# ZhangXiaze/DeepPointMap

Measured on AMD Instinct MI355X. Metric: LiDAR frames/s (encode+match+register), 65 536 pts/frame, higher is better.
Workload: dtype f32 (attention scores K Q^T and P V, Linear / Conv1d (+ LayerNorm) layers with K <= 2048 as exact three-way bf16 splits: 6 bf16 products per fp32 product, fp32 accumulate -- fp32 accuracy, bf16 matrix pipe; all else fp32); 1 GPU; synthetic 64x65536-pt scans per GPU: Encoder.forward + consecutive-frame registration_forward (256x256) + information matrix per frame; points_per_frame=65536, parallelism=frame-sharded x1, one RCCL gather of descriptors+edges per step, weights=procedural (deeppointmap_amd/weights.py), allocator_reserve_gib=16, geometry_waits_for_caller_stream=True

## Files before the change

### deeppointmap_amd/_lib.py

```python
from __future__ import annotations

import ctypes
import os

import torch
from ctypes import c_char_p, c_double, c_int, c_longlong, c_size_t, c_uint, c_void_p

_HERE = os.path.dirname(os.path.abspath(__file__))
LIB_PATH = os.environ.get("DPM_LIB") or os.path.join(_HERE, "libdpm_hip.so")
VERSION_EXPERIMENT = 0x40000000

P, I, D, LL = c_void_p, c_int, c_double, c_longlong

SIGNATURES = {
    "dpm_version": (I, []),
    "dpm_error_string": (c_char_p, [I]),
    "dpm_prepare_points": (I, [P, P, I, I, I, P, P, P]),
    "dpm_to_channel_first": (I, [P, I, I, I, P, P]),
    "dpm_to_channel_first_ld": (I, [P, I, I, I, P, I, P]),
    "dpm_emit_descriptors": (I, [P, P, P, I, I, I, D, P, P, P, P, P]),
    "dpm_nested_levels": (I, [P, P, I, I, I, P, P, P, P, P]),
    "dpm_gather_frames": (I, [P, LL, I, I, I, P, I, P, P]),
    "dpm_fps_workspace_bytes": (c_size_t, [I, I, I]),
    "dpm_fps": (I, [P, P, I, I, I, P, P, P, P, P]),
    "dpm_fps_ex": (I, [P, P, I, I, I, P, P, P, P, I, P]),
    "dpm_fps_start": (I, [P, P, P, I, I, I, P, P, P, P, P]),
    "dpm_knn_workspace_bytes": (c_size_t, [I, I]),
    "dpm_knn_hybrid": (I, [P, P, P, I, I, I, I, D, P, P, P]),
    "dpm_knn_hybrid_reuse": (I, [P, P, P, I, I, I, I, D, P, P, P, P, P]),
    "dpm_knn_build_grid": (I, [P, P, I, I, D, P, P]),
    "dpm_knn_hybrid_prebuilt": (I, [P, P, P, I, I, I, I, D, P, P, P]),
    "dpm_ball_query": (I, [P, P, P, I, I, I, I, D, P, P]),
    "dpm_voxel_sampler_bounds": (I, [P, P, I, I, I, D, D, P, P]),
    "dpm_voxel_sampler_workspace_bytes": (c_size_t, [I, I, LL]),
    "dpm_voxel_sampler_select": (I, [P, P, I, I, I, D, D, P, LL, I, P, I, P, P, P]),
    "dpm_posegraph_optimize": (I, [P, I, P, P, P, P, I, I, P, P, P]),
    "dpm_host_topk_replay": (I, [P, I, I, I, P]),
    "dpm_host_sort_replay": (I, [P, I, I, P]),
    "dpm_group_mlp_max": (I, [P, P, P, P, P, P, P, P, I, I, I, I, I, I, D, P, P]),
    "dpm_group_mlp_max_generic": (I, [P, P, P, P, P, P, P, P, I, I, I, I, I, I, D, P, P]),
    "dpm_group_mlp_max_from_xyz": (I, [P, P, P, P, P, P, P, P, P, I, I, I, I, I, I, D, P, P]),
    "dpm_group_gather_ln_max": (I, [P, P, P, P, P, I, P, P, I, I, I, I, I, D, P, P]),
    "dpm_group_gather_ln_max_folded": (I, [P, P, P, P, I, P, P, I, I, I, I, I, D, P, P]),
    "dpm_group_affine_ln_max": (I, [P, P, P, P, P, P, I, P, P, I, I, I, I, I, D, P, P]),
    "dpm_group_gather_ln_max_centred": (I, [P, P, P, P, I, P, P, I, I, I, I, I, D, P, P]),
    "dpm_group_affine_ln_max_centred": (I, [P, P, P, P, P, P, I, P, P, I, I, I, I, I, D, P, P]),
    "dpm_linear": (I, [P, I, P, I, P, P, I, P, I, I, I, I, I, P]),
    "dpm_linear_batched": (I, [P, I, LL, P, I, LL, P, P, I, LL, P, I, LL, I, I, I, I, I, P]),
    "dpm_split_bf16x3": (I, [P, LL, P, P]),
    "dpm_linear_bf16x3": (I, [P, I, P, I, LL, P, P, I, P, I, I, I, I, I, P]),
    "dpm_linear_bf16x3_rank3": (I, [P, I, P, I, LL, P, P, I, P, I, I, I, I, I, P, P, I, D, P]),
    "dpm_linear_layernorm_bf16x3": (I, [P, I, P, I, LL, P, P, P, P, P, P, I, I, I, I, I, P]),
    "dpm_pwconv_pair_bf16x3": (I, [P, I, P, LL, P, P, P, P, LL, P, P, P, P, P, I, I, I, P]),
    "dpm_decoder_tail_bf16x3": (I, [P, P, P, P, I, I, P, LL, P, P, P, P, LL, P, P, LL, P, P, P, P]),
    "dpm_layernorm": (I, [P, I, P, P, P, P, P, I, I, I, I, P]),
    "dpm_linear_layernorm": (I, [P, I, P, I, P, P, P, P, P, P, I, I, I, I, I, P]),
    "dpm_three_interp_cat": (I, [P, P, P, P, P, I, I, I, I, I, P, P]),
    "dpm_posemb": (I, [P, I, P, I, I, I, P, P]),
    "dpm_attention": (I, [P, I, LL, P, I, LL, P, I, LL, P, I, LL, I, I, I, I, I, P]),
    "dpm_attention_shifted": (I, [P, I, LL, P, I, LL, P, I, LL, P, I, LL, I, I, I, I, I, I, P]),
    "dpm_attention_masked": (I, [P, I, LL, P, I, LL, P, I, LL, P, I, LL, I, I, I, I, I, I, P, P]),
    "dpm_attention_indexed": (I, [P, I, LL, P, I, LL, P, I, LL, P, I, LL, I, I, I, I, I, I, P, P]),
    "dpm_attention_split_workspace_bytes": (c_size_t, [I, I, I, I, I]),
    "dpm_attention_planes_bytes": (c_size_t, [I, I, I]),
    "dpm_attention_planes": (I, [P, I, LL, P, P, I, LL, I, I, I, I, I, P, P]),
    "dpm_linear_bf16x3_kvplanes": (I, [P, I, P, I, LL, P, P, I, I, I, I, I, I, I, P, P]),
    "dpm_attention_split": (I, [P, I, LL, P, I, LL, P, I, LL, P, I, LL, I, I, I, I, I, I, I, P, P]),
    "dpm_l2_normalize": (I, [P, I, I, P, P]),
    "dpm_match_workspace_bytes": (c_size_t, [I, I, I, I]),
    "dpm_match_topk": (I, [P, P, I, I, I, I, D, I, P, P, P, P]),
    "dpm_pairing_workspace_bytes": (c_size_t, [I, I, I]),
    "dpm_dual_softmax_topk": (I, [P, I, I, I, D, I, P, P, P, P]),
    "dpm_gather_pairs": (I, [P, P, P, I, I, I, I, I, P, P, P, P]),
    "dpm_mean_rows": (I, [P, I, I, I, P, I, P]),
    "dpm_kabsch_workspace_bytes": (c_size_t, [I, I]),
    "dpm_corr_kabsch": (I, [P, P, I, LL, P, I, LL, P, P, P, I, I, D, I, D, P, P, P, I, P]),
    "dpm_preprocess_workspace_bytes": (c_size_t, [LL]),
    "dpm_preprocess_scan": (I, [P, I, I, D, D, D, D, LL, P, P, I, P, P, P]),
    "dpm_knn_self_workspace_bytes": (c_size_t, [I]),
    "dpm_knn_self": (I, [P, I, I, D, P, P, P, P, P]),
    "dpm_point_normals": (I, [P, I, D, P, P, P]),
    "dpm_lowpass_similarity": (I, [P, P, I, I, I, P, P]),
    "dpm_stat_filter": (I, [P, I, D, I, D, P, P, P, P, P, P]),
    "dpm_filter_dc_workspace_bytes": (c_size_t, [I, I]),
    "dpm_outlier_filter_dc": (I, [P, P, P, I, I, D, D, D, P, P, P, P, P]),
    "dpm_lowpass_filter_dc": (I, [P, P, P, I, D, I, D, I, D, D, P, P, P, P, P]),
    "dpm_augment_workspace_bytes": (c_size_t, [I, LL]),
    "dpm_ground_filter": (I, [P, P, P, I, I, I, D, D, I, P, P, P, P, P]),
    "dpm_voxel_select": (I, [P, P, P, I, D, I, LL, P, P, P, P, P]),
    "dpm_mask_select": (I, [P, P, P, I, I, D, D, P, D, P, I, P, P, P, P, P]),
    "dpm_points_affine": (I, [P, P, I, I, P, P, P]),
    "dpm_points_deskew": (I, [P, P, P, I, I, P, I, I, P, D, P]),
    "dpm_gather_points": (I, [P, P, P, I, P, I, I, P, P, P, P]),
    "dpm_pack_frames": (I, [P, P, P, I, I, P, P, P, P]),
    "dpm_ingest_frames": (I, [P, P, LL, I, I, I, P, P, P, P, P]),
    "dpm_map_tile": (I, [P, P, P, P, I, I, I, P, P]),
    "dpm_infomat_workspace_bytes": (c_size_t, [I, I, I]),
    "dpm_information_matrix": (I, [P, I, P, I, P, D, P, P, P]),
    "dpm_information_matrix_batched": (I, [P, I, P, P, I, P, I, D, P, I, P, P]),
    "dpm_infomat_build_grids": (I, [P, I, P, I, D, P, P]),
    "dpm_infomat_search_grids": (I, [P, I, P, P, I, P, I, D, P, I, P, P]),
    "dpm_icp_workspace_bytes": (c_size_t, [I, I]),
    "dpm_icp_refine_batched": (I, [P, I, I, P, P, P, P, I, P, I, P, P, I, D, D, P, P, P, P, P, P, P, P, P]),
    "dpm_voxel_map_workspace_bytes": (c_size_t, [LL]),
    "dpm_voxel_map_init": (I, [LL, P, P]),
    "dpm_voxel_map_bounds": (I, [P, P, P, I, LL, P, P]),
    "dpm_voxel_map_insert": (I, [P, P, P, I, LL, LL, LL, D, D, D, D, P, P]),
    "dpm_voxel_map_finish": (I, [LL, P, P]),
    "dpm_voxel_map_emit": (I, [P, LL, D, D, D, D, P, P, I, P]),
    "dpm_reg_loss_pairs": (I, [P, P, I, I, I, D, P, P, P, P, P]),
    "dpm_reg_loss_workspace_bytes": (c_size_t, [I, I, I, I]),
    "dpm_reg_loss_forward": (I, [P, P, P, P, P, P, P, P, I, I, I, I, D, D, I, P, P, P, P, P, P]),
    "dpm_reg_loss_backward": (I, [P, P, P, P, I, I, I, I, D, D, I, P, P, P, P, P, P]),
    "dpm_attention_train_workspace_bytes": (c_size_t, [I, I, I, I]),
    "dpm_attention_train_forward": (I, [P, I, LL, P, I, LL, P, I, LL, P, I, LL, P, I, I, I, I, I, P, P]),
    "dpm_attention_train_backward": (I, [P, I, LL, P, I, LL, P, I, LL, P, I, LL, P, P, I, LL, P, P, P, P, I, I, I, I, I, P, P]),
    "dpm_offset_pairs_count": (I, [P, P, P, P, I, I, I, D, P, P, P]),
    "dpm_offset_pairs_fill": (I, [P, P, P, P, I, I, I, D, P, P, P]),
    "dpm_offset_pairs_gather": (I, [P, I, P, I, I, LL, I, P, P]),
    "dpm_offset_pairs_segment_sum": (I, [P, I, P, P, LL, I, P, P]),
    "dpm_group_train_forward": (I, [P, P, P, P, P, I, P, P, I, I, I, I, I, D, P, P, P]),
    "dpm_group_train_workspace_bytes": (c_size_t, [I, I, I, I, I]),
    "dpm_group_train_backward": (I, [P, P, P, P, P, I, P, I, I, I, I, I, D, P, P, P, P, P, P, P, P]),
    "dpm_loop_pool_workspace_bytes": (c_size_t, [I, I, I]),
    "dpm_loop_pool_forward": (I, [P, I, P, P, I, I, I, P, P, P]),
    "dpm_loop_pool_backward": (I, [P, I, P, P, P, I, I, I, P, P, P, P]),
    "dpm_loop_bce_forward": (I, [P, P, I, P, P, P, P]),
    "dpm_dense_train_workspace_bytes": (c_size_t, [LL, I, I]),
    "dpm_dense_train_forward": (I, [P, I, P, I, P, P, P, P, P, LL, I, I, I, P, P, P, P]),
    "dpm_dense_train_backward_rows": (I, [P, P, P, P, P, LL, I, I, P, P, P, P, P, P]),
    "dpm_dense_train_backward_gemm": (I, [P, P, I, P, I, LL, I, I, P, P, P, P, P]),
    "dpm_map_poses": (I, [P, P, P, P, P, I, I, I, P, P, P]),
    "dpm_map_assemble_fwd": (I, [P, P, P, P, P, I, I, I, I, I, D, P, P, P, P, P, P, P]),
    "dpm_map_assemble_bwd": (I, [P, P, I, I, I, I, I, P, P]),
    "dpm_optim_chunk": (I, []),
    "dpm_optim_step": (I, [I, P, P, I, D, D, D, D, D, D, D, D, I, I, P]),
    "dpm_flat_pack": (I, [P, P, I, P, LL, P]),
    "dpm_flat_unpack": (I, [P, P, I, P, LL, P]),
    "dpm_optim_step_synced": (I, [I, P, P, I, D, D, D, D, D, D, D, D, I, I, P, I, LL, D, P]),
    "dpm_lidar_cull": (I, [P, P, I, P, P, I, D, I, P, P, P, P]),
    "dpm_lidar_cast": (I, [P, P, P, I, I, P, I, I, D, D, P, P, P, P]),
    "dpm_lidar_cull_sweep": (I, [P, P, I, P, P, P, I, I, D, I, P, P, P, P, P]),
    "dpm_lidar_cast_sweep": (I, [P, P, P, I, I, P, I, I, P, I, D, D, P, P, P, P]),
    "dpm_lidar_emit": (I, [P, P, P, P, I, I, P, P, D, P, P, I, P, P, P, P, P, P]),
    "dpm_scene_distance": (I, [P, I, P, I, D, I, D, D, D, P, P, P]),
    "dpm_cloud_nn_workspace_bytes": (c_size_t, [I, I]),
    "dpm_cloud_nn": (I, [P, I, P, I, D, D, D, D, P, P, P, P]),
    "dpm_distance_stats_workspace_bytes": (c_size_t, [I, I, I]),
    "dpm_distance_stats": (I, [P, I, P, P, I, I, P, I, D, P, P, P]),
    "dpm_local_map_bytes": (c_size_t, [I, I]),
    "dpm_local_map_init": (I, [P, I, I, P]),
    "dpm_local_map_insert": (I, [P, I, I, I, D, P, P, P, P, I, P, c_uint, D, D, P]),
    "dpm_local_map_prune": (I, [P, I, I, I, D, P, P, D, P]),
    "dpm_local_map_insert_frames": (I, [P, I, I, I, D, P, P, P, I, I, P, P, P, I, P, D, D, D, P]),
    "dpm_local_map_register": (I, [P, I, I, I, D, P, P, P, I, P, P, P, I, D, D, D, P, P, P, P, P, P, P, P, P, P]),
    "dpm_local_map_export": (I, [P, I, I, I, P, P, P, P, P, I, P]),
    "dpm_local_map_planes": (I, [P, I, I, I, D, P, D, P, P, P]),
    "dpm_local_map_register_planes": (I, [P, I, I, I, D, P, P, P, I, D, P, P, I, P, P, P, I, D, D, D, P, P, P, P, P, P, P, P, P,
                                          P]),
    "dpm_tsdf_bytes": (c_size_t, [I]),
    "dpm_tsdf_init": (I, [P, I, P]),
    "dpm_tsdf_integrate": (I, [P, I, D, P, P, P, I, P, D, D, D, D, P]),
    "dpm_tsdf_integrate_frames": (I, [P, I, D, P, P, P, I, I, P, P, I, D, D, D, D, P]),
    "dpm_tsdf_integrate_planes": (I, [P, I, D, P, P, P, P, I, P, D, D, D, D, D, P]),
    "dpm_tsdf_integrate_planes_frames": (I, [P, I, D, P, P, P, P, I, I, P, P, I, D, D, D, D, D, P]),
    "dpm_tsdf_carve": (I, [P, I, D, P, P, P, I, P, D, D, D, D, I, D, P]),
    "dpm_tsdf_carve_frames": (I, [P, I, D, P, P, P, I, I, P, P, I, D, D, D, D, I, D, P]),
    "dpm_tsdf_export": (I, [P, I, P, P, P, P, I, P]),
    "dpm_tsdf_surface": (I, [P, I, D, I, P, P, P, P, P, I, P]),
    "dpm_tsdf_mesh": (I, [P, I, D, I, P, P, P, P, I, P]),
    "dpm_tsdf_sample": (I, [P, I, D, P, P, P, I, P, I, P, P, P, P]),
    "dpm_tsdf_register_scratch_bytes": (c_size_t, [I]),
    "dpm_tsdf_register": (I, [P, I, D, P, D, I, D, P, P, I, P, P, P, I, D, D, D, P, P, P, P, P, P, P, P, P]),
    "dpm_tsdf_blocks_bytes": (c_size_t, [I]),
    "dpm_tsdf_blocks": (I, [P, I, I, P, I, P]),
    "dpm_tsdf_raycast": (I, [P, I, D, P, P, I, P, I, P, I, D, D, D, I, P, P, P, P]),
    "dpm_scan_context_build": (I, [P, P, I, I, I, D, D, D, P, P, P, P, P, P]),
    "dpm_scan_context_build_batched": (I, [P, P, I, I, I, I, D, D, D, P, P, P, P, P, P]),
    "dpm_scan_context_search_workspace_bytes": (c_size_t, [I, I, I]),
    "dpm_scan_context_search": (I, [P, P, I, P, P, I, P, I, I, I, P, P, P, P, P]),
}


class DpmError(RuntimeError):
    pass


_lib = None


def load() -> ctypes.CDLL:
    global _lib
    if _lib is None:
        if not os.path.exists(LIB_PATH):
            raise DpmError(
                f"{LIB_PATH} not found: the HIP extension is not built. "
                "Run `python deeppointmap_amd/csrc/build.py` (there is no CPU fallback)."
            )
        lib = ctypes.CDLL(LIB_PATH)
        for name, (res, args) in SIGNATURES.items():
            fn = getattr(lib, name)
            fn.restype, fn.argtypes = res, args
        if lib.dpm_version() & VERSION_EXPERIMENT:
            import sys
            print(f"deeppointmap_amd: {LIB_PATH} is an EXPERIMENTAL build (-DDPM_EXPERIMENT): its kernels read DPM_* "
                  "measurement switches from the environment, some of which skip work -- not for results", file=sys.stderr)
        _lib = lib
# ... 15 lines not shown
```

### deeppointmap_amd/csrc/build.py

```python
#!/usr/bin/env python3
import os
import subprocess
import sys
from concurrent.futures import ThreadPoolExecutor

HERE = os.path.dirname(os.path.abspath(__file__))
OUT = os.path.join(os.path.dirname(HERE), "libdpm_hip.so")
ARCH = "gfx950"
COMMON = ["--offload-arch=" + ARCH, "-O3", "-std=c++17", "-fPIC", "-Wall", "-Wno-unused-function",
          "-ffp-contract=off", "-Xclang", "-target-feature", "-Xclang", "-packed-fp32-ops"]
SOURCES = {
    "fps.hip": [],
    "fps_tree.hip": [],
    "knn.hip": [],
    "encoder_ops.hip": [],
    "gemm.hip": [],
    "gemm_b3.hip": [],
    "group_mlp.hip": [],
    "decoder_ops.hip": [],
    "match.hip": [],
    "infomat.hip": [],
    "icp.hip": [],
    "preprocess.hip": [],
    "voxel_sample.hip": [],
    "posegraph.hip": [],
    "voxel_map.hip": [],
    "reg_loss.hip": [],
    "attention_train.hip": [],
    "offset_pairs.hip": [],
    "group_train.hip": [],
    "loop_head_train.hip": [],
    "dense_train.hip": [],
    "augment.hip": [],
    "map_assemble.hip": [],
    "optim.hip": [],
    "ingest.hip": [],
    "lidar_sim.hip": [],
    "map_eval.hip": [],
    "deskew.hip": [],
    "gn_one.hip": [],
    "local_map.hip": [],
    "scan_context.hip": [],
    "tsdf_map.hip": [],
}


def _stale(target, deps):
    if not os.path.exists(target):
        return True
    t = os.path.getmtime(target)
    return any(os.path.getmtime(d) > t for d in deps)


def build(force=False, verbose=False, flags=(), out=None, only=None):
    hipcc = os.environ.get("HIPCC", "/opt/rocm/bin/hipcc")
    objdir = os.path.join(HERE, "build") if out is None else os.path.join(HERE, "build", os.path.basename(out) + ".d")
    OUT = globals()["OUT"] if out is None else out
    os.makedirs(objdir, exist_ok=True)
    headers = [os.path.join(HERE, h) for h in os.listdir(HERE) if h.endswith(".h")]
    headers.append(os.path.join(os.path.dirname(os.path.dirname(HERE)), "include", "dpm_hip.h"))
    jobs = []
    for src, extra in SOURCES.items():
        s = os.path.join(HERE, src)
        o = os.path.join(objdir, src.replace(".hip", ".o"))
        if force or _stale(o, [s] + headers):
            jobs.append([hipcc, *COMMON, *extra, *(flags if only is None or src in only else ()), "-c", s, "-o", o])

    def run(cmd):
        if verbose:
            print(" ".join(cmd), flush=True)
        subprocess.check_call(cmd)

    with ThreadPoolExecutor(max_workers=4) as ex:
        list(ex.map(run, jobs))
    objs = [os.path.join(objdir, s.replace(".hip", ".o")) for s in SOURCES]
    if force or jobs or _stale(OUT, objs):
        staged = OUT + ".unlinted"
        run([hipcc, "--offload-arch=" + ARCH, "-shared", "-fPIC", "-o", staged, *objs])
        sys.path.insert(0, HERE)
        import isa_lint
        try:
            if out is None:
                isa_lint.check(staged)
            elif verbose:
                print("packed fp32 instructions:", isa_lint.packed_fp32(staged))
        except BaseException:
            os.remove(staged)
            raise
        os.replace(staged, OUT)
    return OUT


def build_abi_smoke(verbose=False):
    hipcc = os.environ.get("HIPCC", "/opt/rocm/bin/hipcc")
    root = os.path.dirname(os.path.dirname(HERE))
    src = os.path.join(root, "tests", "c", "abi_gpu_smoke.cpp")
    exe = os.path.join(HERE, "build", "abi_gpu_smoke")
    if not os.path.exists(src):
        return None
    if _stale(exe, [src, OUT, os.path.join(root, "include", "dpm_hip.h")]):
        cmd = [hipcc, "--offload-arch=" + ARCH, "-O2", "-ffp-contract=off", "-I" + os.path.join(root, "include"), src, "-o", exe,
               "-L" + os.path.dirname(OUT), "-ldpm_hip", "-Wl,-rpath,$ORIGIN/../.."]
        if verbose:
            print(" ".join(cmd), flush=True)
        subprocess.check_call(cmd)
    return exe


if __name__ == "__main__":
    if "--out" in sys.argv:
        i = sys.argv.index("--out")
        rest, only = sys.argv[i + 2:], None
        if rest[:1] == ["--only"]:
            only, rest = set(rest[1].split(",")), rest[2:]
            assert only <= set(SOURCES), only
        print(build(verbose=True, flags=tuple(rest), out=os.path.abspath(sys.argv[i + 1]), only=only))
        sys.exit(0)
    print(build(force="--force" in sys.argv, verbose=True))
    print(build_abi_smoke(verbose=True))
```

### deeppointmap_amd/csrc/gemm_b3.hip

```cpp
#include "dpm_common.h"
#include <type_traits>

namespace {

using bf16x8 = __attribute__((ext_vector_type(8))) __bf16;
using f32x4 = __attribute__((ext_vector_type(4))) float;
using u32x4 = __attribute__((ext_vector_type(4))) unsigned;
using u32x2 = __attribute__((ext_vector_type(2))) unsigned;

__device__ __forceinline__ float b3_act(float v, int act) {
    if (act == DPM_ACT_RELU) return fmaxf(v, 0.f);
    if (act == DPM_ACT_SIGMOID) return 1.f / (1.f + __expf(-v));
    return v;
}

__global__ __launch_bounds__(256) void split_bf16x3_kernel(const float *__restrict__ W, long long n, uint16_t *__restrict__ planes) {
    const long long i = (long long)blockIdx.x * 256 + threadIdx.x;
    if (i >= n) return;
    unsigned h, m, l;
    split3(W[i], h, m, l);
    planes[i] = (uint16_t)(h >> 16), planes[n + i] = (uint16_t)(m >> 16), planes[2 * n + i] = (uint16_t)(l >> 16);
}

#ifndef DPM_B3_WIDE
#define DPM_B3_WIDE 1024
#endif
#ifndef DPM_B3_DEEP
#define DPM_B3_DEEP 256
#endif
constexpr int B3_KT = 32, B3_LD = B3_KT;

struct KvPlanes {
    uint16_t *p;
    int col0, tokens, heads;
};

template <int BM, int BN, bool XVEC, int PF, bool KVP>
__device__ __forceinline__ void gemm_b3_body(const float *__restrict__ X, int ldx, const uint16_t *__restrict__ Wp, int ldw,
                                             long long plane, const float *__restrict__ bias,
                                             const float *__restrict__ res, int ldr, float *__restrict__ out, int ldo,
                                             int R, int Cin, int Cout, int act, const float *__restrict__ r3x,
                                             const float *__restrict__ r3w, int ldr3, float r3s, KvPlanes kv) {
    constexpr int LDC = BN + 4, MB = BM / 32, NB = BN / 32, PX = BM / 32, WT = BN * 4, PW = (WT + 255) / 256;
    constexpr int SM0 = 3 * (BM + BN) * B3_LD, SM1 = 2 * BM * LDC, SM = SM0 > SM1 ? SM0 : SM1;
    __shared__ __attribute__((aligned(16))) uint16_t smem[SM];
    uint16_t (*Xs)[BM][B3_LD] = reinterpret_cast<uint16_t (*)[BM][B3_LD]>(smem);
    uint16_t (*Ws)[BN][B3_LD] = reinterpret_cast<uint16_t (*)[BN][B3_LD]>(smem + 3 * BM * B3_LD);
    const int t = threadIdx.x, lane = t & 63, w = t >> 6, wm = w >> 1, wn = w & 1;
    int by = blockIdx.y, bx = blockIdx.x;
    if ((gridDim.y & 7) == 0 && gridDim.y >= 64) {
        const unsigned L = blockIdx.y * gridDim.x + blockIdx.x, xcd = L & 7, slot = L >> 3;
        by = (int)((slot / gridDim.x) * 8 + xcd), bx = (int)(slot % gridDim.x);
    }
    const int row0 = by * BM, col0 = bx * BN;
    const int xr_ = t >> 3, xk = (t & 7) * 4, wr_ = min(t >> 2, BN - 1), wk = (t & 3) * 8;
    const float *xp[PX];
#pragma unroll
    for (int p = 0; p < PX; ++p) xp[p] = X + (size_t)min(row0 + p * 32 + xr_, R - 1) * ldx + xk;
    const uint16_t *wp[PW];
#pragma unroll
    for (int p = 0; p < PW; ++p) wp[p] = Wp + (size_t)min(col0 + p * 64 + wr_, Cout - 1) * ldw + wk;
    auto load_x = [&](const float *p) {
        if (XVEC) return *reinterpret_cast<const f32x4 *>(p);
        return f32x4{p[0], p[1], p[2], p[3]};
    };
    f32x4 xv[PF][PX];
    u32x4 wv[PF][PW][3];
#pragma unroll
    for (int d = 0; d < PF; ++d) {
        const int kd = min(d * B3_KT, Cin - B3_KT);
#pragma unroll
        for (int p = 0; p < PX; ++p) xv[d][p] = load_x(xp[p] + kd);
#pragma unroll
        for (int p = 0; p < PW; ++p)
#pragma unroll
            for (int pl = 0; pl < 3; ++pl) wv[d][p][pl] = *reinterpret_cast<const u32x4 *>(wp[p] + pl * plane + kd);
    }
    f32x4 acc[MB][NB];
#pragma unroll
    for (int i = 0; i < MB; ++i)
#pragma unroll
        for (int j = 0; j < NB; ++j) acc[i][j] = f32x4{0.f, 0.f, 0.f, 0.f};
    const int fr = lane & 15, fk = (lane >> 4) * 8;
    auto stage_x = [&](const f32x4 &v, int r) {
        unsigned h0, m0, l0, h1, m1, l1, h2, m2, l2, h3, m3, l3;
        split3(v[0], h0, m0, l0), split3(v[1], h1, m1, l1), split3(v[2], h2, m2, l2), split3(v[3], h3, m3, l3);
        *reinterpret_cast<u32x2 *>(&Xs[0][r][b3_col(r, xk)]) = u32x2{pack2(h0, h1), pack2(h2, h3)};
        *reinterpret_cast<u32x2 *>(&Xs[1][r][b3_col(r, xk)]) = u32x2{pack2(m0, m1), pack2(m2, m3)};
        *reinterpret_cast<u32x2 *>(&Xs[2][r][b3_col(r, xk)]) = u32x2{pack2(l0, l1), pack2(l2, l3)};
    };
    for (int kb = 0; kb < Cin; kb += B3_KT * PF)
#pragma unroll
    for (int d = 0; d < PF; ++d) {
        const int k0 = kb + d * B3_KT;
        if (PF > 1 && k0 >= Cin) break;
#pragma unroll
        for (int p = 0; p < PX; ++p) stage_x(xv[d][p], p * 32 + xr_);
        if (WT >= 256 || t < WT) {
#pragma unroll
            for (int p = 0; p < PW; ++p)
#pragma unroll
                for (int pl = 0; pl < 3; ++pl) *reinterpret_cast<u32x4 *>(&Ws[pl][p * 64 + wr_][b3_col(wr_, wk)]) = wv[d][p][pl];
        }
        __syncthreads();
        {
            const int kn = min(k0 + PF * B3_KT, Cin - B3_KT);
#pragma unroll
            for (int p = 0; p < PX; ++p) xv[d][p] = load_x(xp[p] + kn);
#pragma unroll
            for (int p = 0; p < PW; ++p)
#pragma unroll
                for (int pl = 0; pl < 3; ++pl) wv[d][p][pl] = *reinterpret_cast<const u32x4 *>(wp[p] + pl * plane + kn);
        }
        bf16x8 a[3][NB], b[3][MB];
#pragma unroll
        for (int pl = 0; pl < 3; ++pl) {
#pragma unroll
            for (int j = 0; j < NB; ++j) a[pl][j] = *reinterpret_cast<const bf16x8 *>(&Ws[pl][wn * (BN / 2) + j * 16 + fr][b3_col(fr, fk)]);
#pragma unroll
            for (int i = 0; i < MB; ++i) b[pl][i] = *reinterpret_cast<const bf16x8 *>(&Xs[pl][wm * (BM / 2) + i * 16 + fr][b3_col(fr, fk)]);
        }
#define DPM_B3(PWQ, PXQ)                                                                                   \
    _Pragma("unroll") for (int i = 0; i < MB; ++i) _Pragma("unroll") for (int j = 0; j < NB; ++j)        \
        acc[i][j] = __builtin_amdgcn_mfma_f32_16x16x32_bf16(a[PWQ][j], b[PXQ][i], acc[i][j], 0, 0, 0)
        DPM_B3(1, 1);
        DPM_B3(2, 0);
        DPM_B3(0, 2);
        DPM_B3(1, 0);
        DPM_B3(0, 1);
        DPM_B3(0, 0);
#undef DPM_B3
        __syncthreads();
    }
    float *ct = reinterpret_cast<float *>(smem);
#pragma unroll
    for (int i = 0; i < MB; ++i)
#pragma unroll
        for (int j = 0; j < NB; ++j)
            *reinterpret_cast<float4 *>(&ct[(wm * (BM / 2) + i * 16 + (lane & 15)) * LDC + wn * (BN / 2) + j * 16 + (lane >> 4) * 4]) =
                make_float4(acc[i][j][0], acc[i][j][1], acc[i][j][2], acc[i][j][3]);
    __syncthreads();
    if (KVP && BM == 64 && BN % 32 == 0 && col0 >= kv.col0) {
        const int E = kv.heads * 32, colk = col0 - kv.col0, isV = colk >= E ? 1 : 0, head0 = (colk - isV * E) >> 5;
        const int sq_ = row0 / kv.tokens, kt = (row0 - sq_ * kv.tokens) >> 6, ntile = kv.tokens >> 6;
#pragma unroll 1
        for (int hh = 0; hh < BN / 32; ++hh) {
            uint16_t *img = kv.p + ((((size_t)sq_ * kv.heads + head0 + hh) * ntile + kt) * 2 + isV) * 6144;
            const float *bh = bias ? bias + col0 + hh * 32 : nullptr;
#pragma unroll
            for (int p = 0; p < 2; ++p) {
                const int e = t + p * 256;
                if (!isV) {
                    const int kr = e >> 3, c4 = (e & 7) * 4;
                    float4 v = *reinterpret_cast<const float4 *>(&ct[kr * LDC + hh * 32 + c4]);
                    if (bh) {
                        const float4 bv = *reinterpret_cast<const float4 *>(bh + c4);
                        v.x += bv.x, v.y += bv.y, v.z += bv.z, v.w += bv.w;
                    }
                    unsigned h0, m0, l0, h1, m1, l1, h2, m2, l2, h3, m3, l3;
                    split3(v.x, h0, m0, l0), split3(v.y, h1, m1, l1), split3(v.z, h2, m2, l2), split3(v.w, h3, m3, l3);
                    uint16_t *o = img + kr * 32 + b3_col(kr, c4);
                    *reinterpret_cast<u32x2 *>(o) = u32x2{pack2(h0, h1), pack2(h2, h3)};
                    *reinterpret_cast<u32x2 *>(o + 2048) = u32x2{pack2(m0, m1), pack2(m2, m3)};
                    *reinterpret_cast<u32x2 *>(o + 4096) = u32x2{pack2(l0, l1), pack2(l2, l3)};
                } else {
                    const int d = e & 31, slot0 = (e >> 5) * 4;
                    const int key0 = 32 * (slot0 >> 5) + 16 * ((slot0 & 7) >> 2) + 4 * ((slot0 >> 3) & 3);
                    const float b = bh ? bh[d] : 0.f;
                    unsigned hq[4], mq[4], lq[4];
#pragma unroll
                    for (int q = 0; q < 4; ++q) split3(ct[(key0 + q) * LDC + hh * 32 + d] + b, hq[q], mq[q], lq[q]);
                    uint16_t *o = img + d * 64 + (((((slot0 >> 3) ^ (d >> 1)) & 7) << 3) | (slot0 & 7));
                    *reinterpret_cast<u32x2 *>(o) = u32x2{pack2(hq[0], hq[1]), pack2(hq[2], hq[3])};
                    *reinterpret_cast<u32x2 *>(o + 2048) = u32x2{pack2(mq[0], mq[1]), pack2(mq[2], mq[3])};
                    *reinterpret_cast<u32x2 *>(o + 4096) = u32x2{pack2(lq[0], lq[1]), pack2(lq[2], lq[3])};
                }
            }
        }
        return;
    }
    constexpr int TPR = BN / 4, RPS = 256 / TPR;
    const int cr = t / TPR, cc = (t % TPR) * 4, c = col0 + cc;
    if (c < Cout) {
// ... 50 lines not shown
template <int BM, int BN, int WGM, int WGN>
__global__ __launch_bounds__(64 * WGM * WGN) void gemm_ln_b3_kernel(const float *__restrict__ X, int ldx, const uint16_t *__restrict__ Wp,
                                                                   int ldw, long long plane, const float *__restrict__ bias,
                                                                   const float *__restrict__ pre, const float *__restrict__ gamma,
                                                                   const float *__restrict__ beta, const float *__restrict__ post,
                                                                   float *__restrict__ out, int ldo, int R, int Cin, int act) {
    constexpr int NP = 1;
    constexpr int BNP = BN / NP;
    constexpr int T = 64 * WGM * WGN, WM = BM / WGM, WN = BNP / WGN, MB = WM / 16, NB = WN / 16, LDC = BN + 4;
    constexpr int XF = BM * 8, PX = (XF + T - 1) / T;
    constexpr int WF = BNP * 4, PW = (WF + T - 1) / T;
    constexpr int SM0 = 3 * (BM + BNP) * B3_LD, SM1 = 2 * BM * LDC, SM = SM0 > SM1 ? SM0 : SM1;
    static_assert(MB >= 1 && NB >= 1 && BN % NP == 0 && WM % 16 == 0 && WN % 16 == 0, "tile shape");
    __shared__ __attribute__((aligned(16))) uint16_t smem[SM];
    uint16_t (*Xs)[BM][B3_LD] = reinterpret_cast<uint16_t (*)[BM][B3_LD]>(smem);
    uint16_t (*Ws)[BNP][B3_LD] = reinterpret_cast<uint16_t (*)[BNP][B3_LD]>(smem + 3 * BM * B3_LD);
    const int t = threadIdx.x, lane = t & 63, w = t >> 6, wm = w / WGN, wn = w % WGN;
    const int row0 = blockIdx.x * BM;
    const float *xp[PX];
    int xrow[PX], xk[PX];
#pragma unroll
    for (int p = 0; p < PX; ++p) {
        const int g = min(p * T + t, XF - 1);
        xrow[p] = g >> 3, xk[p] = (g & 7) * 4;
        xp[p] = X + (size_t)min(row0 + xrow[p], R - 1) * ldx + xk[p];
    }
    const uint16_t *wp[PW];
    int wrow[PW], wk[PW];
#pragma unroll
    for (int p = 0; p < PW; ++p) {
        const int g = min(p * T + t, WF - 1);
        wrow[p] = g >> 2, wk[p] = (g & 3) * 8;
        wp[p] = Wp + (size_t)wrow[p] * ldw + wk[p];
    }
    f32x4 xv[PX];
    u32x4 wv[PW][3];
#pragma unroll
    for (int p = 0; p < PX; ++p) xv[p] = *reinterpret_cast<const f32x4 *>(xp[p]);
#pragma unroll
    for (int p = 0; p < PW; ++p)
#pragma unroll
        for (int pl = 0; pl < 3; ++pl) wv[p][pl] = *reinterpret_cast<const u32x4 *>(wp[p] + pl * plane);
    f32x4 acc[NP][MB][NB];
#pragma unroll
    for (int ps = 0; ps < NP; ++ps)
#pragma unroll
        for (int i = 0; i < MB; ++i)
#pragma unroll
            for (int j = 0; j < NB; ++j) acc[ps][i][j] = f32x4{0.f, 0.f, 0.f, 0.f};
    const int fr = lane & 15, fk = (lane >> 4) * 8;
#pragma unroll
    for (int ps = 0; ps < NP; ++ps)
    for (int k0 = 0; k0 < Cin; k0 += B3_KT) {
#pragma unroll
        for (int p = 0; p < PX; ++p) {
            if (XF % T == 0 || p * T + t < XF) {
                unsigned h0, m0, l0, h1, m1, l1, h2, m2, l2, h3, m3, l3;
                split3(xv[p][0], h0, m0, l0), split3(xv[p][1], h1, m1, l1), split3(xv[p][2], h2, m2, l2), split3(xv[p][3], h3, m3, l3);
                *reinterpret_cast<u32x2 *>(&Xs[0][xrow[p]][b3_col(xrow[p], xk[p])]) = u32x2{pack2(h0, h1), pack2(h2, h3)};
                *reinterpret_cast<u32x2 *>(&Xs[1][xrow[p]][b3_col(xrow[p], xk[p])]) = u32x2{pack2(m0, m1), pack2(m2, m3)};
                *reinterpret_cast<u32x2 *>(&Xs[2][xrow[p]][b3_col(xrow[p], xk[p])]) = u32x2{pack2(l0, l1), pack2(l2, l3)};
            }
        }
#pragma unroll
        for (int p = 0; p < PW; ++p) {
            if (WF % T == 0 || p * T + t < WF) {
#pragma unroll
                for (int pl = 0; pl < 3; ++pl) *reinterpret_cast<u32x4 *>(&Ws[pl][wrow[p]][b3_col(wrow[p], wk[p])]) = wv[p][pl];
            }
        }
        __syncthreads();
        {
            const bool wrap = k0 + B3_KT >= Cin && ps + 1 < NP;
            const int kn = wrap ? 0 : min(k0 + B3_KT, Cin - B3_KT);
            const size_t wo = (size_t)(wrap ? ps + 1 : ps) * BNP * ldw + kn;
#pragma unroll
            for (int p = 0; p < PX; ++p) xv[p] = *reinterpret_cast<const f32x4 *>(xp[p] + kn);
#pragma unroll
            for (int p = 0; p < PW; ++p)
#pragma unroll
                for (int pl = 0; pl < 3; ++pl) wv[p][pl] = *reinterpret_cast<const u32x4 *>(wp[p] + pl * plane + wo);
        }
        bf16x8 a[3][NB], b[3][MB];
#pragma unroll
        for (int pl = 0; pl < 3; ++pl) {
#pragma unroll
            for (int j = 0; j < NB; ++j) a[pl][j] = *reinterpret_cast<const bf16x8 *>(&Ws[pl][wn * WN + j * 16 + fr][b3_col(fr, fk)]);
#pragma unroll
            for (int i = 0; i < MB; ++i) b[pl][i] = *reinterpret_cast<const bf16x8 *>(&Xs[pl][wm * WM + i * 16 + fr][b3_col(fr, fk)]);
        }
#define DPM_B3(PWQ, PXQ)                                                                                   \
    _Pragma("unroll") for (int i = 0; i < MB; ++i) _Pragma("unroll") for (int j = 0; j < NB; ++j)        \
        acc[ps][i][j] = __builtin_amdgcn_mfma_f32_16x16x32_bf16(a[PWQ][j], b[PXQ][i], acc[ps][i][j], 0, 0, 0)
        DPM_B3(1, 1);
        DPM_B3(2, 0);
        DPM_B3(0, 2);
        DPM_B3(1, 0);
        DPM_B3(0, 1);
        DPM_B3(0, 0);
#undef DPM_B3
        __syncthreads();
    }
    float *ct = reinterpret_cast<float *>(smem);
#pragma unroll
    for (int ps = 0; ps < NP; ++ps)
#pragma unroll
        for (int i = 0; i < MB; ++i)
#pragma unroll
            for (int j = 0; j < NB; ++j)
                *reinterpret_cast<float4 *>(&ct[(wm * WM + i * 16 + (lane & 15)) * LDC + ps * BNP + wn * WN + j * 16 + (lane >> 4) * 4]) =
                    make_float4(acc[ps][i][j][0], acc[ps][i][j][1], acc[ps][i][j][2], acc[ps][i][j][3]);
    __syncthreads();
    constexpr int G = BN / 4, RPS = T / G;
    const int cr = t / G, cc = (t % G) * 4;
    const float4 bv = bias ? *reinterpret_cast<const float4 *>(bias + cc) : make_float4(0.f, 0.f, 0.f, 0.f);
    const float4 g4 = *reinterpret_cast<const float4 *>(gamma + cc), b4 = *reinterpret_cast<const float4 *>(beta + cc);
    auto gsum = [](float v) {
#pragma unroll
        for (int off = 1; off < G; off <<= 1) v += __shfl_xor(v, off, 64);
        return v;
    };
#pragma unroll 4
    for (int p = 0; p < BM / RPS; ++p) {
        const int r = row0 + p * RPS + cr, rr = min(r, R - 1);
        float4 v = *reinterpret_cast<const float4 *>(&ct[(p * RPS + cr) * LDC + cc]);
        v.x += bv.x, v.y += bv.y, v.z += bv.z, v.w += bv.w;
        if (pre) {
            const float4 pv = *reinterpret_cast<const float4 *>(pre + (size_t)rr * BN + cc);
            v.x += pv.x, v.y += pv.y, v.z += pv.z, v.w += pv.w;
        }
        const float mu = gsum((v.x + v.y) + (v.z + v.w)) / (float)BN;
        v.x -= mu, v.y -= mu, v.z -= mu, v.w -= mu;
        const float rs = rsqrtf(gsum(fmaf(v.x, v.x, fmaf(v.y, v.y, fmaf(v.z, v.z, v.w * v.w)))) / (float)BN + 1e-5f);
        float4 o = make_float4(fmaf(v.x * rs, g4.x, b4.x), fmaf(v.y * rs, g4.y, b4.y), fmaf(v.z * rs, g4.z, b4.z),
                               fmaf(v.w * rs, g4.w, b4.w));
        if (post) {
            const float4 pv = *reinterpret_cast<const float4 *>(post + (size_t)rr * BN + cc);
            o.x += pv.x, o.y += pv.y, o.z += pv.z, o.w += pv.w;
        }
        o.x = b3_act(o.x, act), o.y = b3_act(o.y, act), o.z = b3_act(o.z, act), o.w = b3_act(o.w, act);
        if (r < R) *reinterpret_cast<float4 *>(out + (size_t)r * ldo + cc) = o;
    }
}

struct TailArgs {
    const float *a, *pre, *post;
    float *out;
    const uint16_t *w[3];
    long long plane[3];
    const float *bias[3];
    const float *g2, *be2, *g3, *be3;
    int R;
};
constexpr int DT_BM = 64, DT_C = 256, DT_T = 512, DT_NK = DT_C / B3_KT, DT_LDC = DT_C + 4;
#ifndef DPM_TAIL_STASH
#define DPM_TAIL_STASH 2
#endif
constexpr int DT_NS = DPM_TAIL_STASH, DT_OPER = 3 * (DT_BM + DT_C) * B3_LD;
__device__ __forceinline__ f32x4 *dt_stash(uint16_t *smem, int kt) {
    return reinterpret_cast<f32x4 *>(smem + DT_OPER) + (kt - (DT_NK - DT_NS)) * DT_T + threadIdx.x;
}
__device__ __forceinline__ void dt_stash_put(uint16_t *smem, const f32x4 (&v)[DT_NK]) {
#pragma unroll
    for (int kt = DT_NK - DT_NS; kt < DT_NK; ++kt) *dt_stash(smem, kt) = v[kt];
}

template <typename V, typename P>
__device__ __forceinline__ V *dt_at(P *uniform, unsigned bytes) {
    using B = std::conditional_t<std::is_const<P>::value, const char, char>;
    return reinterpret_cast<V *>(reinterpret_cast<B *>(uniform) + bytes);
}
__device__ __forceinline__ long long dt_uniform(long long o) {
    const unsigned lo = __builtin_amdgcn_readfirstlane((unsigned)o), hi = __builtin_amdgcn_readfirstlane((unsigned)((unsigned long long)o >> 32));
    return (long long)(((unsigned long long)hi << 32) | lo);
}
template <int CTRL>
__device__ __forceinline__ float dt_dpp(float v) {
    return __int_as_float(__builtin_amdgcn_update_dpp(__float_as_int(v), __float_as_int(v), CTRL, 0xF, 0xF, false));
}
__device__ __forceinline__ float dt_row_sum(float (&s)[DT_NK]) {
#pragma unroll
    for (int kt = 0; kt < DT_NK; ++kt) {
        s[kt] += dt_dpp<0xB1>(s[kt]);
        s[kt] += dt_dpp<0x4E>(s[kt]);
        s[kt] += dt_dpp<0x141>(s[kt]);
    }
    return ((s[0] + s[1]) + (s[2] + s[3])) + ((s[4] + s[5]) + (s[6] + s[7]));
}
__device__ __forceinline__ void dt_layernorm(f32x4 (&v)[DT_NK], const float *__restrict__ gamma, const float *__restrict__ beta, int sk) {
    float s[DT_NK];
#pragma unroll
    for (int kt = 0; kt < DT_NK; ++kt) s[kt] = (v[kt][0] + v[kt][1]) + (v[kt][2] + v[kt][3]);
    const float mu = dt_row_sum(s) / (float)DT_C;
#pragma unroll
    for (int kt = 0; kt < DT_NK; ++kt) {
        v[kt][0] -= mu, v[kt][1] -= mu, v[kt][2] -= mu, v[kt][3] -= mu;
        s[kt] = fmaf(v[kt][0], v[kt][0], fmaf(v[kt][1], v[kt][1], fmaf(v[kt][2], v[kt][2], v[kt][3] * v[kt][3])));
    }
    const float rs = rsqrtf(dt_row_sum(s) / (float)DT_C + 1e-5f);
#pragma unroll
    for (int kt = 0; kt < DT_NK; ++kt) {
        const f32x4 g4 = *reinterpret_cast<const f32x4 *>(gamma + kt * B3_KT + sk), b4 = *reinterpret_cast<const f32x4 *>(beta + kt * B3_KT + sk);
#pragma unroll
        for (int q = 0; q < 4; ++q) v[kt][q] = fmaf(v[kt][q] * rs, g4[q], b4[q]);
    }
}

__device__ __forceinline__ const u32x4 *dt_wsrc(const uint16_t *__restrict__ Wp, long long plane, int p, int pl, int k0, unsigned wo) {
    return dt_at<const u32x4>(Wp + dt_uniform(pl * plane + p * (DT_T / 4) * DT_C) + k0, wo);
}
__device__ __forceinline__ unsigned dt_woff() { return (unsigned)((threadIdx.x >> 2) * DT_C + (threadIdx.x & 3) * 8) * 2u; }
__device__ __forceinline__ void dt_wtile0(const uint16_t *__restrict__ Wp, long long plane, u32x4 (&wv)[2][3]) {
    const unsigned wo = dt_woff();
#pragma unroll
    for (int p = 0; p < 2; ++p)
#pragma unroll
        for (int pl = 0; pl < 3; ++pl) wv[p][pl] = *dt_wsrc(Wp, plane, p, pl, 0, wo);
}

template <bool XREG, typename Mid>
__device__ __forceinline__ void dt_product(uint16_t *smem, const float *xg, unsigned xo, const f32x4 (&xr)[DT_NK], const uint16_t *__restrict__ Wp,
                                           long long plane, u32x4 (&wv)[2][3], f32x4 (&acc)[2][4], Mid mid) {
    constexpr int WM = 32, WN = 64, MB = 2, NB = 4, PW = 2;
    uint16_t (*Xs)[DT_BM][B3_LD] = reinterpret_cast<uint16_t (*)[DT_BM][B3_LD]>(smem);
    uint16_t (*Ws)[DT_C][B3_LD] = reinterpret_cast<uint16_t (*)[DT_C][B3_LD]>(smem + 3 * DT_BM * B3_LD);
    const int t = threadIdx.x, lane = t & 63, w = t >> 6, wm = w >> 2, wn = w & 3;
    const int sr = t >> 3, sk = (t & 7) * 4, wk = (t & 3) * 8, fr = lane & 15, fk = (lane >> 4) * 8;
    const int wrow = t >> 2;
    const unsigned wo = dt_woff();
    f32x4 xv = f32x4{0.f, 0.f, 0.f, 0.f};
    if (!XREG) xv = *dt_at<const f32x4>(xg, xo);
#pragma unroll
    for (int i = 0; i < MB; ++i)
#pragma unroll
        for (int j = 0; j < NB; ++j) acc[i][j] = f32x4{0.f, 0.f, 0.f, 0.f};
#pragma unroll
    for (int kt = 0; kt < DT_NK; ++kt) {
        {
            const f32x4 x = !XREG ? xv : kt >= DT_NK - DT_NS ? *dt_stash(smem, kt) : xr[kt];
            unsigned h0, m0, l0, h1, m1, l1, h2, m2, l2, h3, m3, l3;
            split3(x[0], h0, m0, l0), split3(x[1], h1, m1, l1), split3(x[2], h2, m2, l2), split3(x[3], h3, m3, l3);
            *reinterpret_cast<u32x2 *>(&Xs[0][sr][b3_col(sr, sk)]) = u32x2{pack2(h0, h1), pack2(h2, h3)};
            *reinterpret_cast<u32x2 *>(&Xs[1][sr][b3_col(sr, sk)]) = u32x2{pack2(m0, m1), pack2(m2, m3)};
            *reinterpret_cast<u32x2 *>(&Xs[2][sr][b3_col(sr, sk)]) = u32x2{pack2(l0, l1), pack2(l2, l3)};
        }
#pragma unroll
        for (int p = 0; p < PW; ++p)
#pragma unroll
            for (int pl = 0; pl < 3; ++pl) *reinterpret_cast<u32x4 *>(&Ws[pl][p * (DT_T / 4) + wrow][b3_col(wrow, wk)]) = wv[p][pl];
        __syncthreads();
        if (kt + 1 < DT_NK) {
            const int kn = (kt + 1) * B3_KT;
            unsigned wok = wo;
            asm volatile("" : "+v"(wok));
            if (!XREG) xv = *dt_at<const f32x4>(xg + kn, xo);
#pragma unroll
            for (int p = 0; p < PW; ++p)
#pragma unroll
                for (int pl = 0; pl < 3; ++pl) wv[p][pl] = *dt_wsrc(Wp, plane, p, pl, kn, wok);
        }
        mid(kt);
        bf16x8 b[3][MB];
#pragma unroll
        for (int pl = 0; pl < 3; ++pl)
#pragma unroll
            for (int i = 0; i < MB; ++i) b[pl][i] = *reinterpret_cast<const bf16x8 *>(&Xs[pl][wm * WM + i * 16 + fr][b3_col(fr, fk)]);
#pragma unroll
        for (int j = 0; j < NB; ++j) {
            bf16x8 a[3];
#pragma unroll
            for (int pl = 0; pl < 3; ++pl) a[pl] = *reinterpret_cast<const bf16x8 *>(&Ws[pl][wn * WN + j * 16 + fr][b3_col(fr, fk)]);
#define DPM_B3(PWQ, PXQ) \
    _Pragma("unroll") for (int i = 0; i < MB; ++i) acc[i][j] = __builtin_amdgcn_mfma_f32_16x16x32_bf16(a[PWQ], b[PXQ][i], acc[i][j], 0, 0, 0)
            DPM_B3(1, 1);
            DPM_B3(2, 0);
            DPM_B3(0, 2);
            DPM_B3(1, 0);
            DPM_B3(0, 1);
            DPM_B3(0, 0);
#undef DPM_B3
        }
        __syncthreads();
    }
}

template <typename Mid>
__device__ __forceinline__ void dt_restage(uint16_t *smem, const f32x4 (&acc)[2][4], f32x4 (&v)[DT_NK], Mid mid) {
    float *ct = reinterpret_cast<float *>(smem);
    int t = threadIdx.x;
    asm volatile("" : "+v"(t));
    const int lane = t & 63, w = t >> 6, wm = w >> 2, wn = w & 3, sr = t >> 3, sk = (t & 7) * 4;
#pragma unroll
    for (int i = 0; i < 2; ++i)
#pragma unroll
        for (int j = 0; j < 4; ++j)
            *reinterpret_cast<f32x4 *>(&ct[(wm * 32 + i * 16 + (lane & 15)) * DT_LDC + wn * 64 + j * 16 + (lane >> 4) * 4]) = acc[i][j];
    mid();
    __syncthreads();
#pragma unroll
    for (int kt = 0; kt < DT_NK; ++kt) v[kt] = *reinterpret_cast<const f32x4 *>(&ct[sr * DT_LDC + kt * B3_KT + sk]);
    __syncthreads();
}

__device__ __forceinline__ void dt_add_bias(f32x4 (&v)[DT_NK], const float *__restrict__ bias, int sk) {
#pragma unroll
    for (int kt = 0; kt < DT_NK; ++kt) {
        const f32x4 bv = bias ? *reinterpret_cast<const f32x4 *>(bias + kt * B3_KT + sk) : f32x4{0.f, 0.f, 0.f, 0.f};
        v[kt] += bv;
    }
}

template <bool ZREG>
__global__ __launch_bounds__(DT_T) __attribute__((amdgpu_waves_per_eu(4, 4))) void decoder_tail_b3_kernel(TailArgs A) {
    constexpr int SM0 = DT_OPER + DT_NS * DT_T * 8, SM1 = 2 * DT_BM * DT_LDC, SM = SM0 > SM1 ? SM0 : SM1;
    __shared__ __attribute__((aligned(16))) uint16_t smem[SM];
    const int t = threadIdx.x, sr = t >> 3, sk = (t & 7) * 4;
    const int row0 = blockIdx.x * DT_BM, r = row0 + sr;
    const long long base = dt_uniform((long long)row0 * DT_C);
    const unsigned ro = (unsigned)(min(sr, A.R - 1 - row0) * DT_C + sk) * 4u;
    const float *ga = A.a + base, *gpre = A.pre + base, *gpost = (A.post ? A.post : A.pre) + base;
    float *gout = A.out + base;
    f32x4 acc[2][4], v[DT_NK], z[DT_NK];
    u32x4 wv[2][3];
    dt_wtile0(A.w[0], A.plane[0], wv);
    dt_product<false>(smem, ga, ro, v, A.w[0], A.plane[0], wv, acc, [&](int kt) {
        if (kt == DT_NK - 1) {
#pragma unroll
            for (int k2 = 0; k2 < DT_NK; ++k2) z[k2] = *dt_at<const f32x4>(gpre + k2 * B3_KT, ro);
        }
    });
    dt_restage(smem, acc, v, [&] { dt_wtile0(A.w[1], A.plane[1], wv); });
    dt_add_bias(v, A.bias[0], sk);
#pragma unroll
    for (int kt = 0; kt < DT_NK; ++kt) v[kt] += z[kt];
    dt_layernorm(v, A.g2, A.be2, sk);
    if (ZREG) {
#pragma unroll
        for (int kt = 0; kt < DT_NK; ++kt) z[kt] = v[kt];
    } else if (r < A.R) {
#pragma unroll
        for (int kt = 0; kt < DT_NK; ++kt) *dt_at<f32x4>(gout + kt * B3_KT, ro) = v[kt];
    }
    dt_stash_put(smem, v);
    dt_product<true>(smem, nullptr, 0u, v, A.w[1], A.plane[1], wv, acc, [](int) {});
    dt_restage(smem, acc, v, [&] { dt_wtile0(A.w[2], A.plane[2], wv); });
    dt_add_bias(v, A.bias[1], sk);
#pragma unroll
    for (int kt = 0; kt < DT_NK; ++kt)
#pragma unroll
        for (int q = 0; q < 4; ++q) v[kt][q] = fmaxf(v[kt][q], 0.f);
    dt_stash_put(smem, v);
    dt_product<true>(smem, nullptr, 0u, v, A.w[2], A.plane[2], wv, acc, [&](int kt) {
        if (!ZREG && kt == DT_NK - 1) {
#pragma unroll
            for (int k2 = 0; k2 < DT_NK; ++k2) z[k2] = *dt_at<const f32x4>(gout + k2 * B3_KT, ro);
        }
    });
    f32x4 pv[DT_NK];
    dt_restage(smem, acc, v, [&] {
        if (A.post) {
#pragma unroll
            for (int kt = 0; kt < DT_NK; ++kt) pv[kt] = *dt_at<const f32x4>(gpost + kt * B3_KT, ro);
        }
    });
    dt_add_bias(v, A.bias[2], sk);
#pragma unroll
    for (int kt = 0; kt < DT_NK; ++kt) v[kt] += z[kt];
    dt_layernorm(v, A.g3, A.be3, sk);
    if (A.post) {
#pragma unroll
        for (int kt = 0; kt < DT_NK; ++kt) v[kt] += pv[kt];
    }
    if (r < A.R) {
#pragma unroll
        for (int kt = 0; kt < DT_NK; ++kt) *dt_at<f32x4>(gout + kt * B3_KT, ro) = v[kt];
    }
}


#ifndef DPM_PW_GRID
#define DPM_PW_GRID 768
#endif
constexpr int PW_C = 32, PW_H = 128;
__device__ __forceinline__ float pw_rows4_sum(float v) {
    auto a = __builtin_amdgcn_permlane32_swap(__float_as_uint(v), __float_as_uint(v), false, false);
    v = __uint_as_float(a[0]) + __uint_as_float(a[1]);
    auto b = __builtin_amdgcn_permlane16_swap(__float_as_uint(v), __float_as_uint(v), false, false);
    return __uint_as_float(b[0]) + __uint_as_float(b[1]);
}
__global__ __launch_bounds__(256) void pwconv_pair_b3_kernel(const float *__restrict__ X, int ldx, const uint16_t *__restrict__ W1p,
                                                            long long plane1, const float *__restrict__ b1,
                                                            const float *__restrict__ g1, const float *__restrict__ be1,
                                                            const uint16_t *__restrict__ W2p, long long plane2,
                                                            const float *__restrict__ b2, const float *__restrict__ g2,
                                                            const float *__restrict__ be2, const float *__restrict__ post,
                                                            float *__restrict__ out, int R, int tiles_per_wave) {
    __shared__ __attribute__((aligned(16))) uint16_t W1s[3][PW_H][PW_C];
    __shared__ __attribute__((aligned(16))) uint16_t W2s[3][PW_H / 32][PW_C][32];
    __shared__ __attribute__((aligned(16))) float vec1[3][PW_H];
    __shared__ __attribute__((aligned(16))) float vec2[3][PW_C];
    const int t = threadIdx.x, lane = t & 63, w = t >> 6, g = lane >> 4, fr = lane & 15;
    for (int e = t; e < 3 * PW_H * 4; e += 256) {
        const int pl = e / (PW_H * 4), r = (e / 4) % PW_H, c = (e & 3) * 8;
        *reinterpret_cast<u32x4 *>(&W1s[pl][r][b3_col(r, c)]) = *reinterpret_cast<const u32x4 *>(W1p + pl * plane1 + r * PW_C + c);
    }
    for (int e = t; e < 3 * PW_C * 16; e += 256) {
        const int pl = e / (PW_C * 16), r = (e / 16) % PW_C, c = (e & 15) * 8;
        *reinterpret_cast<u32x4 *>(&W2s[pl][c >> 5][r][b3_col(r, c & 31)]) =
            *reinterpret_cast<const u32x4 *>(W2p + pl * plane2 + r * PW_H + c);
    }
    if (t < PW_H) vec1[0][t] = b1 ? b1[t] : 0.f, vec1[1][t] = g1[t], vec1[2][t] = be1[t];
    if (t < PW_C) vec2[0][t] = b2 ? b2[t] : 0.f, vec2[1][t] = g2[t], vec2[2][t] = be2[t];
    __syncthreads();
    const long long tile0 = ((long long)blockIdx.x * 4 + w) * tiles_per_wave;
    f32x4 nx0, nx1, np0, np1;
    auto request = [&](long long r0) {
        const int r = (int)min(r0 + fr, (long long)R - 1);
        const float *xp = X + (size_t)r * ldx + 8 * g;
        nx0 = *reinterpret_cast<const f32x4 *>(xp), nx1 = *reinterpret_cast<const f32x4 *>(xp + 4);
        np0 = post ? *reinterpret_cast<const f32x4 *>(post + (size_t)r * PW_C + 4 * g) : f32x4{0.f, 0.f, 0.f, 0.f};
        np1 = post ? *reinterpret_cast<const f32x4 *>(post + (size_t)r * PW_C + 16 + 4 * g) : f32x4{0.f, 0.f, 0.f, 0.f};
    };
    request(min(tile0 * 16, (long long)R - 1));
    for (int it = 0; it < tiles_per_wave; ++it) {
        const long long row0 = (tile0 + it) * 16;
        if (row0 >= R) break;
        const int row = (int)min(row0 + fr, (long long)R - 1);
        const f32x4 x0 = nx0, x1 = nx1, p0 = np0, p1 = np1;
        request(min(row0 + 16, (long long)R - 1));
        bf16x8 xb[3];
        {
            unsigned hh[8], mm[8], ll[8];
#pragma unroll
            for (int e = 0; e < 4; ++e) split3(x0[e], hh[e], mm[e], ll[e]), split3(x1[e], hh[4 + e], mm[4 + e], ll[4 + e]);
            xb[0] = __builtin_bit_cast(bf16x8, u32x4{pack2(hh[0], hh[1]), pack2(hh[2], hh[3]), pack2(hh[4], hh[5]), pack2(hh[6], hh[7])});
            xb[1] = __builtin_bit_cast(bf16x8, u32x4{pack2(mm[0], mm[1]), pack2(mm[2], mm[3]), pack2(mm[4], mm[5]), pack2(mm[6], mm[7])});
            xb[2] = __builtin_bit_cast(bf16x8, u32x4{pack2(ll[0], ll[1]), pack2(ll[2], ll[3]), pack2(ll[4], ll[5]), pack2(ll[6], ll[7])});
        }
        f32x4 h[PW_H / 16];
#pragma unroll
        for (int j = 0; j < PW_H / 16; j += 2) {
            bf16x8 a[2][3];
#pragma unroll
            for (int jj = 0; jj < 2; ++jj)
#pragma unroll
                for (int pl = 0; pl < 3; ++pl)
                    a[jj][pl] = *reinterpret_cast<const bf16x8 *>(&W1s[pl][(j + jj) * 16 + fr][b3_col(fr, 8 * g)]);
            h[j] = h[j + 1] = f32x4{0.f, 0.f, 0.f, 0.f};
#define DPM_PW1(PWQ, PXQ)                                                                             \
    _Pragma("unroll") for (int jj = 0; jj < 2; ++jj)                                                  \
        h[j + jj] = __builtin_amdgcn_mfma_f32_16x16x32_bf16(a[jj][PWQ], xb[PXQ], h[j + jj], 0, 0, 0)
            DPM_PW1(1, 1);
            DPM_PW1(2, 0);
            DPM_PW1(0, 2);
            DPM_PW1(1, 0);
            DPM_PW1(0, 1);
            DPM_PW1(0, 0);
#undef DPM_PW1
        }
        float sum = 0.f;
#pragma unroll
        for (int j = 0; j < PW_H / 16; ++j) {
            const f32x4 bv = *reinterpret_cast<const f32x4 *>(&vec1[0][16 * j + 4 * g]);
// ... 210 lines not shown
```

### deeppointmap_amd/decoder.py

```python
from __future__ import annotations

import copy
import threading
from typing import Dict, Tuple, Union

import torch
import torch.nn.functional as F
from torch.utils.checkpoint import checkpoint

from . import knobs, ops
from .params import ParamTree, decoder_shapes

HEADS = 8


class Decoder(ParamTree):
    def __init__(self, args):
        super().__init__(decoder_shapes(args))
        self.args = args
        self.decoder_cfg = args.decoder
        self.in_channel = self.decoder_cfg.in_channel
        self.model_channel = self.decoder_cfg.model_channel
        self.attention_layers = self.decoder_cfg.attention_layers
        self.tau = args.loss.tau
        self._dim_t: Dict[str, torch.Tensor] = {}
        self.fused_match = knobs.FUSED_MATCH
        self.stack_sides = True
        self.dedup_frames = knobs.DEDUP_FRAMES
        self.graph_min_hits = 2
        self.graph_max = 6
        self._graphs: Dict[tuple, dict] = {}
        self._graph_lock = threading.Lock()
        self._stamp_params = None
        self.train_checkpoint_rows = 8192
        self.eval()

    def __deepcopy__(self, memo):
        new = self.__class__.__new__(self.__class__)
        memo[id(self)] = new
        for k, v in self.__dict__.items():
            if k == "_graphs":
                new.__dict__[k] = {}
            elif k == "_stamp_params":
                new.__dict__[k] = None
            elif k == "_graph_lock":
                new.__dict__[k] = threading.Lock()
            else:
                new.__dict__[k] = copy.deepcopy(v, memo)
        return new

    @property
    def device(self) -> torch.device:
        return self.p("projection.weight").device

    def _dimt(self, dev: torch.device) -> torch.Tensor:
        key = str(dev)
        if key not in self._dim_t:
            F = self.model_channel // 3 // 2 * 2
            i = torch.arange(F, dtype=torch.float32)
            self._dim_t[key] = (10000 ** (2 * torch.div(i, 2, rounding_mode="trunc") / F)).to(dev)
        return self._dim_t[key]

    def _lin(self, key: str, x, act=ops.ACT_NONE, residual=None):
        return ops.linear(x, self.p(key + ".weight"), self.p(key + ".bias"), act=act, residual=residual)

    def _ln(self, key: str, x, post=None):
        return ops.layernorm(x, self.p(key + ".weight"), self.p(key + ".bias"), post=post)

    def _lin_ln(self, lin: str, ln: str, x, residual, post=None):
        return ops.linear_layernorm(x, self.p(lin + ".weight"), self.p(lin + ".bias"), self.p(ln + ".weight"),
                                    self.p(ln + ".bias"), pre=residual, post=post)

    def _block_tail(self, pre: str, a, z1, post=None):
        ca, n2, m0, m2, n3 = pre + ".cross_attn.out_proj", pre + ".norm2", pre + ".mlp.0", pre + ".mlp.2", pre + ".norm3"
        out = ops.decoder_tail(a, z1, self.p(ca + ".weight"), self.p(ca + ".bias"), self.p(n2 + ".weight"), self.p(n2 + ".bias"),
                               self.p(m0 + ".weight"), self.p(m0 + ".bias"), self.p(m2 + ".weight"), self.p(m2 + ".bias"),
                               self.p(n3 + ".weight"), self.p(n3 + ".bias"), post)
        if out is not None:
            return out
        z2 = self._lin_ln(ca, n2, a, z1)
        return self._lin_ln(m2, n3, self._lin(m0, z2, ops.ACT_RELU), z2, post)

    def _stage(self, desc: torch.Tensor, dev) -> Tuple[torch.Tensor, torch.Tensor, int, int]:
        d = desc.to(device=dev, dtype=torch.float32).contiguous()
        B, C, M = d.shape
        if C != self.in_channel + 3:
            raise ValueError(f"descriptor must have {self.in_channel + 3} rows, got {C}")
        t = ops.to_channel_first(d, row_multiple=4)
        return t.as_strided((B * M, C), (t.stride(1), 1), t.storage_offset()), B, M

    def _self_attn(self, pre: str, xp, B, M, norm: str = None, post=None, mask=None):
        E = self.model_channel
        a = ops.qkv_attention(xp, self.p(pre + ".in_proj_weight"), self.p(pre + ".in_proj_bias"), B, M, HEADS) if mask is None else None
        if a is None:
            qkv = ops.linear(xp, self.p(pre + ".in_proj_weight"), self.p(pre + ".in_proj_bias"))
            a = ops.attention(qkv[:, :E], qkv[:, E:2 * E], qkv[:, 2 * E:], B, M, M, HEADS, key_mask=mask)
        if norm is not None:
            return self._lin_ln(pre + ".out_proj", norm, a, xp, post)
        return ops.linear(a, self.p(pre + ".out_proj.weight"), self.p(pre + ".out_proj.bias"), residual=xp)

    def _cross_attn(self, pre: str, xq, xkv, B, M, N, norm: str = None, mask=None, tail=None):
        E = self.model_channel
        w, b = self.p(pre + ".in_proj_weight"), self.p(pre + ".in_proj_bias")
        q = ops.linear(xq, w[:E], b[:E])
        kv = ops.linear(xkv, w[E:], b[E:])
        a = ops.attention(q, kv[:, :E], kv[:, E:], B, M, N, HEADS, key_mask=mask)
        if tail is not None:
            return self._block_tail(tail[0], a, xq, tail[1])
        if norm is not None:
            return self._lin_ln(pre + ".out_proj", norm, a, xq)
        return ops.linear(a, self.p(pre + ".out_proj.weight"), self.p(pre + ".out_proj.bias"), residual=xq)

    def _descriptor_attention_forward(self, src_descriptor, dst_descriptor, src_padding_mask=None,
                                      dst_padding_mask=None):
        dev = self.device
        ts, B, M = self._stage(src_descriptor, dev)
        td, B2, N = self._stage(dst_descriptor, dev)
        if B != B2:
            raise ValueError("src and dst batch sizes differ")
        ms = md = None
        if src_padding_mask is not None or dst_padding_mask is not None:
            def as_mask(m, L):
                if m is None:
                    return torch.zeros(B, L, dtype=torch.uint8, device=dev)
                m = m.to(dev)
                if tuple(m.shape) != (B, L) or m.dtype != torch.bool:
                    raise ValueError(f"padding mask must be a bool tensor of shape ({B}, {L})")
                return m.contiguous().view(torch.uint8)
            ms, md = as_mask(src_padding_mask, M), as_mask(dst_padding_mask, N)
        C, E = self.in_channel, self.model_channel
        xyz_s, xyz_d = ts[:, C:C + 3], td[:, C:C + 3]
        if M == N:
            x, y = self._attention_layers_joint(ts, td, B, M, mask=None if ms is None else torch.cat([ms, md]))
            return x, xyz_s, y, xyz_d, B, M, N
        if self.stack_sides:
            x, y = self._attention_layers_stacked(ts, td, B, M, N, ms, md)
            return x, xyz_s, y, xyz_d, B, M, N
        ps, pd = ops.posemb(xyz_s, self._dimt(dev), E), ops.posemb(xyz_d, self._dimt(dev), E)
        xp = ops.linear(ts[:, :C], self.p("projection.weight"), self.p("projection.bias"), residual=ps)
        yp = ops.linear(td[:, :C], self.p("projection.weight"), self.p("projection.bias"), residual=pd)
        for l in range(self.attention_layers):
            pre = f"descriptor_attention.{l}"
            last = l == self.attention_layers - 1
            x1 = self._self_attn(pre + ".self_attn", xp, B, M, norm=pre + ".norm1", post=ps, mask=ms)
            y1 = self._self_attn(pre + ".self_attn", yp, B, N, norm=pre + ".norm1", post=pd, mask=md)
            xp = self._cross_attn(pre + ".cross_attn", x1, y1, B, M, N, mask=md, tail=(pre, None if last else ps))
            yp = self._cross_attn(pre + ".cross_attn", y1, x1, B, N, M, mask=ms, tail=(pre, None if last else pd))
        return xp, xyz_s, yp, xyz_d, B, M, N

    def _attention_layers_stacked(self, ts, td, B, M, N, ms=None, md=None):
        C, E, dev = self.in_channel, self.model_channel, self.device
        R1 = B * M
        z_in = torch.cat([ts, td], dim=0)
        pos = ops.posemb(z_in[:, C:C + 3], self._dimt(dev), E)
        zp = ops.linear(z_in[:, :C], self.p("projection.weight"), self.p("projection.bias"), residual=pos)
        for l in range(self.attention_layers):
            pre = f"descriptor_attention.{l}"
            last = l == self.attention_layers - 1
            sa, ca = pre + ".self_attn", pre + ".cross_attn"
            qkv = ops.linear(zp, self.p(sa + ".in_proj_weight"), self.p(sa + ".in_proj_bias"))
            a = torch.empty(zp.shape[0], E, device=dev, dtype=torch.float32)
            ops.attention(qkv[:R1, :E], qkv[:R1, E:2 * E], qkv[:R1, 2 * E:], B, M, M, HEADS, out=a[:R1], key_mask=ms)
            ops.attention(qkv[R1:, :E], qkv[R1:, E:2 * E], qkv[R1:, 2 * E:], B, N, N, HEADS, out=a[R1:], key_mask=md)
            z1 = self._lin_ln(sa + ".out_proj", pre + ".norm1", a, zp, pos)
            qkv = ops.linear(z1, self.p(ca + ".in_proj_weight"), self.p(ca + ".in_proj_bias"))
            a = torch.empty(zp.shape[0], E, device=dev, dtype=torch.float32)
            ops.attention(qkv[:R1, :E], qkv[R1:, E:2 * E], qkv[R1:, 2 * E:], B, M, N, HEADS, out=a[:R1], key_mask=md)
            ops.attention(qkv[R1:, :E], qkv[:R1, E:2 * E], qkv[:R1, 2 * E:], B, N, M, HEADS, out=a[R1:], key_mask=ms)
            zp = self._block_tail(pre, a, z1, None if last else pos)
        return zp[:R1], zp[R1:]

    def _attention_layers_joint(self, ts, td, B, M, frames=None, mask=None):
        C, E, R = self.in_channel, self.model_channel, B * M
        dev = self.device
        if frames is not None:
            tu, sidx, didx = frames
            U = tu.shape[0] // M
            pos_u = ops.posemb(tu[:, C:C + 3], self._dimt(dev), E)
            zu = ops.linear(tu[:, :C], self.p("projection.weight"), self.p("projection.bias"), residual=pos_u)
            pre = "descriptor_attention.0"
            z1u = self._self_attn(pre + ".self_attn", zu, U, M, norm=pre + ".norm1", post=pos_u)
            order = sidx if didx is None else torch.cat([sidx, didx])
            pos = ops.gather_frames(pos_u, order, M, E).view(2 * R, E)
            z1_first = ops.gather_frames(z1u, order, M, E).view(2 * R, E)
            ca0 = pre + ".cross_attn"
            a_first = qkv_u = None
            if self.dedup_frames and E // HEADS == 32 and mask is None:
                a_first = ops.qkv_attention(z1u, self.p(ca0 + ".in_proj_weight"), self.p(ca0 + ".in_proj_bias"), 2 * B, M, HEADS,
                                            kv_shift=B, seq_index=order)
                if a_first is None:
                    qkv_u = ops.linear(z1u, self.p(ca0 + ".in_proj_weight"), self.p(ca0 + ".in_proj_bias"))
            zp = None
        else:
            z_in = torch.cat([ts, td], dim=0)
            pos = ops.posemb(z_in[:, C:C + 3], self._dimt(dev), E)
            zp = ops.linear(z_in[:, :C], self.p("projection.weight"), self.p("projection.bias"), residual=pos)
            z1_first = qkv_u = a_first = None
        for l in range(self.attention_layers):
            pre = f"descriptor_attention.{l}"
            last = l == self.attention_layers - 1
            if l == 0 and z1_first is not None:
                z1 = z1_first
            else:
                z1 = self._self_attn(pre + ".self_attn", zp, 2 * B, M, norm=pre + ".norm1", post=pos, mask=mask)
            ca = pre + ".cross_attn"
            if l == 0 and z1_first is not None and a_first is not None:
                a = a_first
            elif l == 0 and z1_first is not None and qkv_u is not None:
                a = ops.attention(qkv_u[:, :E], qkv_u[:, E:2 * E], qkv_u[:, 2 * E:], 2 * B, M, M, HEADS, kv_shift=B,
                                  seq_index=order)
            else:
                a = ops.qkv_attention(z1, self.p(ca + ".in_proj_weight"), self.p(ca + ".in_proj_bias"), 2 * B, M, HEADS,
                                      kv_shift=B) if mask is None else None
                if a is None:
                    qkv = ops.linear(z1, self.p(ca + ".in_proj_weight"), self.p(ca + ".in_proj_bias"))
                    a = ops.attention(qkv[:, :E], qkv[:, E:2 * E], qkv[:, 2 * E:], 2 * B, M, M, HEADS, kv_shift=B, key_mask=mask)
            zp = self._block_tail(pre, a, z1, None if last else pos)
        return zp[:R], zp[R:]

    def train(self, mode: bool = True):
        was = self.training
        super().train(mode)
        loop = self.train_stage == "loop_detection"
        for name, p in self._flat.items():
            p.requires_grad_(bool(mode) and (("loop" in name) == loop))
        if was and not mode:
            self.invalidate_caches()
        return self

    def _train_layer(self, l: int, z, pos, B: int, M: int, N: int, ms, md):
        E, R1 = self.model_channel, B * M
        pre = f"descriptor_attention.{l}"
        nrm = lambda n: (self.p(f"{pre}.{n}.weight"), self.p(f"{pre}.{n}.bias"))
        zp = z + pos
        qkv = self._dense(zp, self.p(pre + ".self_attn.in_proj_weight"), self.p(pre + ".self_attn.in_proj_bias"))
        a = torch.cat([ops.attention_train(qkv[:R1, :E], qkv[:R1, E:2 * E], qkv[:R1, 2 * E:], B, M, M, HEADS, ms),
                       ops.attention_train(qkv[R1:, :E], qkv[R1:, E:2 * E], qkv[R1:, 2 * E:], B, N, N, HEADS, md)])
        z1 = self._dense_ln(a, *self._w(pre + ".self_attn.out_proj"), *nrm("norm1"), residual=zp, post=pos)
        qkv = self._dense(z1, self.p(pre + ".cross_attn.in_proj_weight"), self.p(pre + ".cross_attn.in_proj_bias"))
        a = torch.cat([ops.attention_train(qkv[:R1, :E], qkv[R1:, E:2 * E], qkv[R1:, 2 * E:], B, M, N, HEADS, md),
                       ops.attention_train(qkv[R1:, :E], qkv[:R1, E:2 * E], qkv[:R1, 2 * E:], B, N, M, HEADS, ms)])
        z2 = self._dense_ln(a, *self._w(pre + ".cross_attn.out_proj"), *nrm("norm2"), residual=z1)
        u = self._dense(z2, *self._w(pre + ".mlp.0"), act=ops.ACT_RELU)
        return self._dense_ln(u, *self._w(pre + ".mlp.2"), *nrm("norm3"), residual=z2)

    def _dense2(self, x, first: str, second: str):
        return self._dense(self._dense(x, *self._w(first), act=ops.ACT_RELU), *self._w(second))

    def forward(self, src_descriptor: torch.Tensor, dst_descriptor: torch.Tensor, src_padding_mask: torch.Tensor = None,
                dst_padding_mask: torch.Tensor = None, gt_Rt: Tuple[torch.Tensor, torch.Tensor] = None):
        assert self.training, "forward is not available during inference!"
        assert gt_Rt is not None, "gt_Rt must be provided during training"
        dev = self._require_gpu()
        C, E = self.in_channel, self.model_channel
        if E // HEADS != ops.ATTENTION_TRAIN_HEAD_DIM or E % HEADS:
            raise ValueError(f"Decoder.forward: model_channel {E} gives heads of width {E / HEADS:g}; the training attention "
                             f"kernels support width {ops.ATTENTION_TRAIN_HEAD_DIM} only (model_channel "
                             f"{ops.ATTENTION_TRAIN_HEAD_DIM * HEADS})")
        for name, d in (("src_descriptor", src_descriptor), ("dst_descriptor", dst_descriptor)):
            if d.dim() != 3 or d.shape[1] != C + 3:
                raise ValueError(f"{name} must be (B, {C + 3}, tokens), got {tuple(d.shape)}")
        src = src_descriptor.to(device=dev, dtype=torch.float32)
        dst = dst_descriptor.to(device=dev, dtype=torch.float32)
        B, _, M = src.shape
        N = dst.shape[2]
        if dst.shape[0] != B:
            raise ValueError("src and dst batch sizes differ")

        def as_mask(m, L, name):
            if m is None:
                return torch.zeros(B, L, dtype=torch.bool, device=dev)
            if tuple(m.shape) != (B, L) or m.dtype != torch.bool:
                raise ValueError(f"{name} must be a bool tensor of shape ({B}, {L})")
            return m.to(dev).contiguous()
        ps, pd = as_mask(src_padding_mask, M, "src_padding_mask"), as_mask(dst_padding_mask, N, "dst_padding_mask")
        gt_R, gt_T = gt_Rt
        if tuple(gt_R.shape) != (B, 3, 3) or tuple(gt_T.shape) != (B, 3, 1):
            raise ValueError(f"gt_Rt must be ((B,3,3), (B,3,1)) with B = {B}, got {tuple(gt_R.shape)}, {tuple(gt_T.shape)}")
        gt_R, gt_T = gt_R.detach().to(device=dev, dtype=torch.float32), gt_T.detach().to(device=dev, dtype=torch.float32)
        with torch.cuda.device(dev):
            ms, md = ps.view(torch.uint8), pd.view(torch.uint8)
            R1 = B * M
            rows = torch.cat([src[:, :C].transpose(1, 2).reshape(R1, C), dst[:, :C].transpose(1, 2).reshape(B * N, C)])
            xyz_s, xyz_d = src[:, C:].detach(), dst[:, C:].detach()
            xyz_rows = torch.cat([xyz_s.transpose(1, 2).reshape(R1, 3), xyz_d.transpose(1, 2).reshape(B * N, 3)])

            def split(t, ch):
                return t[:R1].view(B, M, ch).transpose(1, 2), t[R1:].view(B, N, ch).transpose(1, 2)
            coarse = self._dense2(rows, "coarse_pairing_head.0", "coarse_pairing_head.2")
            pos = ops.posemb(xyz_rows, self._dimt(dev), E)
            z = self._dense(rows, *self._w("projection"))
            recompute = B * (M + N) >= self.train_checkpoint_rows
            for l in range(self.attention_layers):
                if recompute:
                    z = checkpoint(self._train_layer, l, z, pos, B, M, N, ms, md, use_reentrant=False)
                else:
                    z = self._train_layer(l, z, pos, B, M, N, ms, md)
            sim = self._dense2(z, "similarity_head.0", "similarity_head.2")
            src_gt = (gt_R @ xyz_s + gt_T).contiguous()
            pairs = ops.offset_pairs(src_gt, xyz_d.contiguous(), ps, pd, self.args.loss.eps_offset)
            xs, xd = ops.offset_pair_rows(z[:R1], z[R1:], pairs, M, N)
            bi, si, di = pairs[0].long().unbind(1)
            K = bi.numel()
            sp, dp = src_gt.transpose(1, 2)[bi, si], xyz_d.transpose(1, 2)[bi, di]
            src_gt_off = gt_R[bi].transpose(1, 2) @ (dp - sp).unsqueeze(2)
            dst_gt_off = (sp - dp).unsqueeze(2)
            X = torch.cat([torch.cat([xs, xd], dim=1), torch.cat([xd, xs], dim=1)])
            h = self._dense(self._dense(X, *self._w("offset_head.mlp.0"), act=ops.ACT_RELU),
                            *self._w("offset_head.mlp.2"), act=ops.ACT_RELU)
            h = self._dense(h, *self._w("offset_head.mlp.4"), act=ops.ACT_RELU,
                            residual=self._dense(X, *self._w("offset_head.downsample")))
            off = self._dense(h, *self._w("offset_head.head")).unsqueeze(2)
            return [*split(sim, E), *split(coarse, C), off[:K] - src_gt_off, off[K:] - dst_gt_off]

    @staticmethod
    def _num_pairs(num_sample, M: int, N: int) -> int:
        if isinstance(num_sample, int):
            k = num_sample
        elif isinstance(num_sample, float) and num_sample > 1:
            k = int(num_sample)
        elif isinstance(num_sample, float) and 0 < num_sample <= 1:
            k = int(num_sample * (M + N))
        else:
            raise ValueError(f"Argument `num_sample` with value {num_sample} is not supported")
        return k // 2

    def _register(self, src_descriptor, dst_descriptor, num_sample, header_out=None, trace: dict = None, pairs=None,
                  masks=(None, None)):
        if pairs is not None:
            dev = self.device
            sidx, didx = pairs[0], pairs[1]
            order = pairs[2] if len(pairs) > 2 else torch.cat([sidx, didx])
            tu, U, M = self._stage(src_descriptor, dev)
            N, B, C = M, sidx.numel(), self.in_channel
            x, y = self._attention_layers_joint(None, None, B, M, frames=(tu, order, None))
            xyz_sd = ops.gather_frames(tu, order, M, 3, ld=tu.stride(0), offset=C).view(2 * B * M, 3)
            xyz_s, xyz_d = xyz_sd[:B * M], xyz_sd[B * M:]
        else:
            x, xyz_s, y, xyz_d, B, M, N = self._descriptor_attention_forward(src_descriptor, dst_descriptor, *masks)
        E = self.model_channel
        k = self._num_pairs(num_sample, M, N)
        if k < 1:
            res = torch.full((B, ops.RES_HDR), float("nan"), device=x.device, dtype=torch.float32)
            res[:, 13:16] = 0.0
            if header_out is not None:
                header_out.copy_(res)
            return res
        if (M == N and x.is_contiguous() and y.is_contiguous() and
                x.untyped_storage().data_ptr() == y.untyped_storage().data_ptr() and
                y.storage_offset() == x.storage_offset() + x.numel()):
            z = x.as_strided((2 * B * M, E), (E, 1), x.storage_offset())
            ab = ops.l2_normalize(self._lin("similarity_head.2", self._lin("similarity_head.0", z, ops.ACT_RELU)))
            a, b = ab[:B * M], ab[B * M:]
        else:
            a = ops.l2_normalize(self._lin("similarity_head.2", self._lin("similarity_head.0", x, ops.ACT_RELU)))
            b = ops.l2_normalize(self._lin("similarity_head.2", self._lin("similarity_head.0", y, ops.ACT_RELU)))
        if self.fused_match and ops.match_supported(M, N, E, k):
            conf, flat = ops.match_topk(a.view(B, M, E), b.view(B, N, E), self.tau, k)
        else:
            S = ops.similarity_batched(a.view(B, M, E), b.view(B, N, E))
            conf, flat = ops.dual_softmax_topk(S, self.tau, k)
        X, si, di = ops.gather_pairs(x.view(B, M, E), y.view(B, N, E), flat)
        X = X.view(B * 2 * k, 2 * E)
        h = self._lin("offset_head.mlp.2", self._lin("offset_head.mlp.0", X, ops.ACT_RELU), ops.ACT_RELU)
        h = self._lin("offset_head.mlp.4", h, ops.ACT_RELU, residual=self._lin("offset_head.downsample", X))
        off = self._lin("offset_head.head", h)
        res = ops.corr_kabsch(off, xyz_s, xyz_d, si, di, conf, self.args.loss.eps_offset, header_out=header_out, batch=B)
        if trace is not None:
            trace.update(x=x, y=y, conf=conf, flat=flat, src_index=si, dst_index=di, offsets=off)
        return res.view(B, -1)

    @torch.no_grad()
    def registration_forward_batch(self, src_descriptor: torch.Tensor, dst_descriptor: torch.Tensor,
                                   num_sample: Union[int, float] = 0.5, header_out: torch.Tensor = None) -> torch.Tensor:
        dev = self._require_gpu()
        with torch.cuda.device(dev):
            return self._register(src_descriptor, dst_descriptor, num_sample, header_out)

    @torch.no_grad()
    def registration_forward_pairs(self, descriptors: torch.Tensor, src_frame: torch.Tensor, dst_frame: torch.Tensor,
                                   num_sample: Union[int, float] = 0.5, header_out: torch.Tensor = None,
                                   order: torch.Tensor = None) -> torch.Tensor:
        dev = self._require_gpu()
        with torch.cuda.device(dev):
            pairs = (src_frame, dst_frame) if order is None else (src_frame, dst_frame, order)
            return self._register(descriptors, None, num_sample, header_out, pairs=pairs)

    def _weights_stamp(self):
        if self._stamp_params is None:
            self._stamp_params = list(self._flat.values())
        return (self._epoch, ops.derived_generation(), tuple([p._version for p in self._stamp_params]))

    def _graph_entry(self, key, M: int, N: int, num_sample, dev):
        with self._graph_lock:
            e = self._graphs.get(key)
            if e is None:
                e = self._graphs[key] = dict(hits=0, graph=None, used=0)
            e["hits"] += 1
            e["used"] = max((v["used"] for v in self._graphs.values()), default=0) + 1
            if e["graph"] is not None:
                if e["stamp"] == self._weights_stamp():
                    return e
                e["graph"] = None
            if self.graph_min_hits <= 0 or e["hits"] <= self.graph_min_hits or threading.active_count() > 1:
                return None
            self._make_room()
        return self._capture(e, M, N, num_sample, dev)

    def _make_room(self):
        live = [k for k, v in self._graphs.items() if v["graph"] is not None and not v.get("pinned")]
        if len(live) >= self.graph_max:
            old = min(live, key=lambda k: self._graphs[k]["used"])
            self._graphs.pop(old)

    def _capture(self, e: dict, M: int, N: int, num_sample, dev):
        src = torch.zeros(1, self.in_channel + 3, M, device=dev, dtype=torch.float32)
        dst = torch.zeros(1, self.in_channel + 3, N, device=dev, dtype=torch.float32)
        side = torch.cuda.Stream(device=dev)
        side.wait_stream(torch.cuda.current_stream(dev))
        g = torch.cuda.CUDAGraph()
        try:
            with torch.cuda.graph(g, stream=side, capture_error_mode="relaxed"):
                res = self._register(src, dst, num_sample)
        except Exception:
            with self._graph_lock:
                e["hits"] = -(1 << 30)
            return None
        torch.cuda.current_stream(dev).wait_stream(side)
        e.update(graph=g, src=src, dst=dst, res=res, stamp=self._weights_stamp())
        return e

    @torch.no_grad()
    def capture_registration_graphs(self, shapes, copies: int = 1) -> int:
        dev = self._require_gpu()
        if threading.active_count() > 1:
            raise RuntimeError("capture_registration_graphs must run before the process starts its worker threads")
        n = 0
        with torch.cuda.device(dev):
            for M, N, num_sample in shapes:
                k = self._num_pairs(num_sample, M, N)
                if k < 1:
                    continue
                for c in range(max(1, int(copies))):
                    key = (M, N, k, dev.index, None, c)
                    with self._graph_lock:
                        e = self._graphs.get(key)
                        if e is not None and e.get("graph") is not None and e["stamp"] == self._weights_stamp():
                            continue
                        e = self._graphs[key] = dict(hits=0, graph=None, used=0, pinned=True, lock=threading.Lock(), done=None)
                    if self._capture(e, M, N, num_sample, dev) is not None:
                        n += 1
        return n

    def _shared_graph(self, M: int, N: int, k: int, dev):
        first, stamp, c = None, None, 0
        while True:
            e = self._graphs.get((M, N, k, dev.index, None, c))
            if e is None:
                break
            if e.get("graph") is not None:
                stamp = self._weights_stamp() if stamp is None else stamp
                if e["stamp"] == stamp:
                    if e["lock"].acquire(blocking=False):
                        return e
                    first = e if first is None else first
            c += 1
        if first is not None:
            first["lock"].acquire()
        return first

    @torch.no_grad()
    def registration_forward(self, src_descriptor: torch.Tensor, dst_descriptor: torch.Tensor,
                             src_padding_mask=None, dst_padding_mask=None,
                             num_sample: Union[int, float] = 0.5, trace: dict = None, header_out: torch.Tensor = None):
        dev = self._require_gpu()
        batch = not (src_descriptor.ndim == 2 and dst_descriptor.ndim == 2)
        if not batch:
            src_descriptor, dst_descriptor = src_descriptor.unsqueeze(0), dst_descriptor.unsqueeze(0)
        assert src_descriptor.shape[0] == 1, "batch size in inference must be 1"
        with torch.cuda.device(dev):
            entry = None
            plain = (src_padding_mask is None and dst_padding_mask is None and trace is None and header_out is None and
                     src_descriptor.ndim == 3 and dst_descriptor.ndim == 3 and dst_descriptor.shape[0] == 1 and
                     src_descriptor.shape[1] == self.in_channel + 3 == dst_descriptor.shape[1] and
                     isinstance(num_sample, (int, float)) and not torch.cuda.is_current_stream_capturing())
            if plain and self.graph_min_hits > 0:
                M, N = src_descriptor.shape[2], dst_descriptor.shape[2]
                k = self._num_pairs(num_sample, M, N)
                if k >= 1:
                    entry = self._shared_graph(M, N, k, dev)
                    if entry is None:
                        entry = self._graph_entry((M, N, k, dev.index, threading.get_ident()), M, N, num_sample, dev)
            if entry is not None and entry.get("lock") is not None:
                try:
                    st = torch.cuda.current_stream(dev)
                    if entry["done"] is not None:
                        st.wait_event(entry["done"])
                    entry["src"].copy_(src_descriptor, non_blocking=True)
                    entry["dst"].copy_(dst_descriptor, non_blocking=True)
                    entry["graph"].replay()
                    res = entry["res"][0].clone()
                    entry["done"] = st.record_event()
                finally:
                    entry["lock"].release()
            elif entry is not None:
                entry["src"].copy_(src_descriptor, non_blocking=True)
                entry["dst"].copy_(dst_descriptor, non_blocking=True)
                entry["graph"].replay()
                res = entry["res"][0].clone()
            else:
                res = self._register(src_descriptor, dst_descriptor, num_sample, header_out, trace,
                                     masks=(src_padding_mask, dst_padding_mask))[0]
            head = res[:ops.RES_HDR].cpu()
        n_in, rmse = int(head[14]), float(head[12])
        R, T, cf = res[0:9].view(3, 3), res[9:12].view(3, 1), res[ops.RES_HDR:ops.RES_HDR + n_in]
        if trace is not None:
            trace.update(n_corr=int(head[13]), iterations=int(head[15]))
        if not batch:
            return R, T, cf, rmse
# ... 30 lines not shown
```

### deeppointmap_amd/knobs.py

```python
from __future__ import annotations

import os

FPS_ALGO = None
FUSED_LN = True
GEMM_BF16X3 = True
BF16X3_MAX_K = 2048
GEMM_LN_BF16X3 = True
BF16X3_LN_MIN_K = 128
FUSED_LN_SMALL_ROWS = 0
FOLD_GATHER = True
FOLD_MIN_RADIUS = 0.2
CENTRED_GATHER = True
FUSED_PWCONV = True
FUSED_MATCH = True
KV_PLANES = True
DECODER_TAIL_FUSED = True
DEDUP_FRAMES = True

_ENV = {"DPM_FOLD_MIN_RADIUS": ("FOLD_MIN_RADIUS", float), "DPM_KV_PLANES": ("KV_PLANES", lambda v: v != "0"), "DPM_CENTRED_GATHER": ("CENTRED_GATHER", lambda v: v != "0"), "DPM_FPS_ALGO": ("FPS_ALGO", int), "DPM_NO_FUSED_LN": ("FUSED_LN", lambda v: v != "1"),
        "DPM_DEDUP_FRAMES": ("DEDUP_FRAMES", lambda v: v != "0"), "DPM_DECODER_TAIL": ("DECODER_TAIL_FUSED", lambda v: v != "0"), "DPM_GEMM_BF16X3": ("GEMM_BF16X3", lambda v: v == "1"), "DPM_BF16X3_MAX_K": ("BF16X3_MAX_K", int), "DPM_BF16X3_LN_MIN_K": ("BF16X3_LN_MIN_K", int), "DPM_FUSED_LN_SMALL_ROWS": ("FUSED_LN_SMALL_ROWS", int), "DPM_GEMM_LN_BF16X3": ("GEMM_LN_BF16X3", lambda v: v == "1"),
        "DPM_FUSED_MATCH": ("FUSED_MATCH", lambda v: v != "0"), "DPM_FUSED_PWCONV": ("FUSED_PWCONV", lambda v: v != "0"), "DPM_FOLD_GATHER": ("FOLD_GATHER", lambda v: v != "0")}


def env_knobs() -> dict:
    return {k: v for k, v in sorted(os.environ.items()) if k.startswith("DPM_")}


def apply_env() -> dict:
    g = globals()
    for var, (name, conv) in _ENV.items():
        if var in os.environ:
            g[name] = conv(os.environ[var])
    return env_knobs()
```

### deeppointmap_amd/ops.py

```python
from __future__ import annotations

from typing import Optional, Tuple

import ctypes
import threading
import weakref

import torch

from . import _lib, knobs

ACT_NONE, ACT_RELU, ACT_SIGMOID = 0, 1, 2


def _ptr(t: Optional[torch.Tensor]):
    return None if t is None else t.data_ptr()


def _stream(t: torch.Tensor):
    return torch.cuda.current_stream(t.device).cuda_stream


def _chk(t: torch.Tensor, dtype, name: str):
    if not t.is_cuda:
# ... 432 lines not shown
        st = _lib.load().dpm_linear_bf16x3(_ptr(x2), x2.stride(0), planes.data_ptr() + 2 * off, Cin, n, _ptr(bias), _ptr(r2),
                                           Cout if r2 is not None else 0, _ptr(o2), o2.stride(0), x2.shape[0], Cin, Cout, act,
                                           _stream(x))
    if st == -2:
        return None
    _lib.check(st, "dpm_linear_bf16x3")
    return out


def similarity_batched(a: torch.Tensor, b: torch.Tensor) -> torch.Tensor:
    _chk(a, torch.float32, "a"), _chk(b, torch.float32, "b")
    B, M, C = a.shape
    N = b.shape[1]
    out = torch.empty(B, M, N, device=a.device, dtype=torch.float32)
    _lib.check(_lib.load().dpm_linear_batched(_ptr(a), C, M * C, _ptr(b), C, N * C, None, None, 0, 0, _ptr(out), N,
                                              M * N, B, M, C, N, ACT_NONE, _stream(a)), "dpm_linear_batched")
    return out


def layernorm(x: torch.Tensor, gamma: torch.Tensor, beta: torch.Tensor, act: int = ACT_NONE,
              pre: Optional[torch.Tensor] = None, post: Optional[torch.Tensor] = None) -> torch.Tensor:
    _chk(x, torch.float32, "x")
    C = x.shape[-1]
    x2 = x.reshape(-1, C)
    out = torch.empty_like(x)
    for n, t in (("pre", pre), ("post", post)):
        if t is not None:
            _chk(t, torch.float32, n)
            if t.numel() != x.numel():
                raise ValueError(f"{n} must have the shape of x")
    _lib.check(_lib.load().dpm_layernorm(_ptr(x2), C, _ptr(pre), _ptr(gamma), _ptr(beta), _ptr(post), _ptr(out), C,
                                         x2.shape[0], C, act, _stream(x)), "dpm_layernorm")
    return out


FUSED_LN_WIDTHS = (32, 64, 128, 256)
FUSED_LN_MIN_ROWS = 16384


def linear_layernorm(x: torch.Tensor, W: torch.Tensor, bias: Optional[torch.Tensor], gamma: torch.Tensor, beta: torch.Tensor,
                     act: int = ACT_NONE, pre: Optional[torch.Tensor] = None, post: Optional[torch.Tensor] = None) -> torch.Tensor:
    Cout, Cin = W.shape[0], W.shape[1]
    x2 = x.reshape(-1, x.shape[-1])
    if (knobs.GEMM_BF16X3 and knobs.GEMM_LN_BF16X3 and Cin % 32 == 0 and knobs.BF16X3_LN_MIN_K <= Cin <= knobs.BF16X3_MAX_K and Cout % 4 == 0 and W.numel() == Cout * Cin
            and x.dtype == torch.float32):
        wp = _weight_planes(W)
        if wp is not None and (bias is None or bias.data_ptr() % 16 == 0):
            if (Cout in FUSED_LN_WIDTHS and (x2.shape[0] >= FUSED_LN_MIN_ROWS or x2.shape[0] <= knobs.FUSED_LN_SMALL_ROWS)
                    and x2.is_contiguous() and knobs.FUSED_LN):
                planes, off, n = wp
                out = torch.empty(*x.shape[:-1], Cout, device=x.device, dtype=torch.float32)
                for nm, t in (("pre", pre), ("post", post)):
                    if t is not None:
                        _chk(t, torch.float32, nm)
                        if t.numel() != out.numel():
                            raise ValueError(f"{nm} must have the shape of the output")
                st = _lib.load().dpm_linear_layernorm_bf16x3(_ptr(x2), x2.stride(0), planes.data_ptr() + 2 * off, Cin, n, _ptr(bias),
                                                             _ptr(pre), _ptr(gamma), _ptr(beta), _ptr(post), _ptr(out), Cout,
                                                             x2.shape[0], Cin, Cout, act, _stream(x))
                if st == 0:
                    return out
                if st != -2:
                    _lib.check(st, "dpm_linear_layernorm_bf16x3")
            y = linear_bf16x3(x, W, bias, residual=pre)
            if y is not None:
                return layernorm(y, gamma, beta, act=act, post=post)
    if (Cout in FUSED_LN_WIDTHS and x2.shape[0] >= FUSED_LN_MIN_ROWS and W.is_contiguous() and x2.is_contiguous()
            and x.dtype == torch.float32 and Cin % 4 == 0 and knobs.FUSED_LN):
        _chk(W, torch.float32, "W")
        out = torch.empty(*x.shape[:-1], Cout, device=x.device, dtype=torch.float32)
        for n, t in (("pre", pre), ("post", post)):
            if t is not None:
                _chk(t, torch.float32, n)
                if t.numel() != out.numel():
                    raise ValueError(f"{n} must have the shape of the output")
        st = _lib.load().dpm_linear_layernorm(_ptr(x2), x2.stride(0), _ptr(W), Cin, _ptr(bias), _ptr(pre), _ptr(gamma),
                                              _ptr(beta), _ptr(post), _ptr(out), Cout, x2.shape[0], Cin, Cout, act, _stream(x))
        if st == 0:
            return out
        if st != -2:
            _lib.check(st, "dpm_linear_layernorm")
    y = linear(x, W, bias, residual=pre, exact=True)
    return layernorm(y, gamma, beta, act=act, post=post)


def _pwconv_kperm() -> torch.Tensor:
    return torch.tensor([16 * (2 * s + (e >> 2)) + 4 * g + (e & 3) for s in range(4) for g in range(4) for e in range(8)], dtype=torch.long)


def pwconv_pair(x: torch.Tensor, W1, b1, g1, be1, W2, b2, g2, be2, post: Optional[torch.Tensor]) -> Optional[torch.Tensor]:
    C, H = W1.shape[1], W1.shape[0]
    if not (knobs.FUSED_PWCONV and knobs.GEMM_BF16X3 and C == 32 and H == 128 and tuple(W2.shape[:2]) == (C, H) and x.is_cuda
            and x.dtype == torch.float32 and x.is_contiguous() and W1.numel() == C * H and W2.numel() == C * H):
        return None
    wp1 = _weight_planes(W1)
    if wp1 is None or (post is not None and (not post.is_contiguous() or post.numel() != x.numel())):
        return None
    for n, t_ in (("gamma1", g1), ("beta1", be1), ("gamma2", g2), ("beta2", be2)):
        _chk(t_, torch.float32, n)

    def make():
        Wp = W2.reshape(C, H)[:, _pwconv_kperm().to(W2.device)].contiguous()
        planes = torch.empty(3, C * H, device=W2.device, dtype=torch.int16)
        _lib.check(_lib.load().dpm_split_bf16x3(_ptr(Wp), C * H, _ptr(planes), _stream(W2)), "dpm_split_bf16x3")
        planes._dpm_keep = Wp
        return planes
    planes2 = _derived("bf16x3-planes-kperm", (W2,), make)
    planes1, off1, n1 = wp1
    x2 = x.reshape(-1, C)
    out = torch.empty_like(x)
    st = _lib.load().dpm_pwconv_pair_bf16x3(_ptr(x2), C, planes1.data_ptr() + 2 * off1, n1, _ptr(b1), _ptr(g1), _ptr(be1),
                                            planes2.data_ptr(), C * H, _ptr(b2), _ptr(g2), _ptr(be2), _ptr(post), _ptr(out),
                                            x2.shape[0], C, H, _stream(x))
    if st == -2:
        return None
    _lib.check(st, "dpm_pwconv_pair_bf16x3")
    return out


def decoder_tail(a: torch.Tensor, z1: torch.Tensor, Wo, bo, g2, be2, W0, b0, W2, b2, g3, be3,
                 post: Optional[torch.Tensor]) -> Optional[torch.Tensor]:
    C = a.shape[-1]
    if not (knobs.DECODER_TAIL_FUSED and knobs.GEMM_BF16X3 and knobs.GEMM_LN_BF16X3 and knobs.FUSED_LN and C == 256
            and knobs.BF16X3_LN_MIN_K <= C <= knobs.BF16X3_MAX_K and a.is_cuda and a.dtype == torch.float32 and a.dim() == 2
            and a.is_contiguous()):
        return None
    R = a.shape[0]
    if not (R >= FUSED_LN_MIN_ROWS or 1 <= R <= knobs.FUSED_LN_SMALL_ROWS):
        return None
    for t_ in (z1, post):
        if t_ is not None and not (t_.dtype == torch.float32 and t_.is_cuda and t_.is_contiguous() and tuple(t_.shape) == (R, C)):
            return None
    planes = []
    for W, b in ((Wo, bo), (W0, b0), (W2, b2)):
        if tuple(W.shape[:2]) != (C, C) or W.numel() != C * C or (b is not None and b.data_ptr() % 16):
            return None
        wp = _weight_planes(W)
        if wp is None:
            return None
        planes.append(wp)
    for n, t_ in (("gamma2", g2), ("beta2", be2), ("gamma3", g3), ("beta3", be3)):
        _chk(t_, torch.float32, n)
    out = torch.empty(R, C, device=a.device, dtype=torch.float32)
    (po, oo, no), (p0, o0, n0), (p2, o2, n2) = planes
    st = _lib.load().dpm_decoder_tail_bf16x3(_ptr(a), _ptr(z1), _ptr(post), _ptr(out), R, C, po.data_ptr() + 2 * oo, no, _ptr(bo),
                                             _ptr(g2), _ptr(be2), p0.data_ptr() + 2 * o0, n0, _ptr(b0), p2.data_ptr() + 2 * o2, n2,
                                             _ptr(b2), _ptr(g3), _ptr(be3), _stream(a))
    if st == -2:
        return None
    _lib.check(st, "dpm_decoder_tail_bf16x3")
    return out


def three_interp_cat(xyz1, xyz2, lengths2, fea1, fea2) -> torch.Tensor:
    for n, t in (("xyz1", xyz1), ("xyz2", xyz2), ("fea1", fea1), ("fea2", fea2)):
        _chk(t, torch.float32, n)
    _chk(lengths2, torch.int32, "lengths2")
    B, N, D1 = fea1.shape
    S, D2 = fea2.shape[1], fea2.shape[2]
    out = torch.empty(B, N, D1 + D2, device=fea1.device, dtype=torch.float32)
    _lib.check(_lib.load().dpm_three_interp_cat(_ptr(xyz1), _ptr(xyz2), _ptr(lengths2), _ptr(fea1), _ptr(fea2),
                                                B, N, S, D1, D2, _ptr(out), _stream(fea1)), "dpm_three_interp_cat")
    return out


def _rows2d(t: torch.Tensor, name: str) -> torch.Tensor:
    if t.dtype != torch.float32 or not t.is_cuda or t.dim() != 2 or t.stride(1) != 1:
        raise ValueError(f"{name}: expected a 2-D fp32 GPU tensor with unit column stride")
    return t


def posemb(xyz_rows: torch.Tensor, dim_t: torch.Tensor, emb_dim: int) -> torch.Tensor:
    _rows2d(xyz_rows, "xyz")
    _chk(dim_t, torch.float32, "dim_t")
    R = xyz_rows.shape[0]
    out = torch.empty(R, emb_dim, device=xyz_rows.device, dtype=torch.float32)
    _lib.check(_lib.load().dpm_posemb(_ptr(xyz_rows), xyz_rows.stride(0), _ptr(dim_t), dim_t.numel(), emb_dim, R,
                                      _ptr(out), _stream(out)), "dpm_posemb")
    return out


ATTENTION_SPLIT_MIN_KEYS = 1024
ATTENTION_SPLIT_BLOCKS = 256


def attention_key_splits(B: int, M: int, N: int, heads: int, head_dim: int) -> int:
    if head_dim != 32 or N < ATTENTION_SPLIT_MIN_KEYS:
        return 1
    blocks = -(-M // 64) * heads
    if blocks >= ATTENTION_SPLIT_BLOCKS:
        return 1
    ns = max(1, min(ATTENTION_SPLIT_BLOCKS // blocks, N // 256, 64))
    chunk = -(-N // (64 * ns)) * 64
    return -(-N // chunk)


def attention(q: torch.Tensor, k: torch.Tensor, v: torch.Tensor, B: int, M: int, N: int, heads: int = 8,
              out: Optional[torch.Tensor] = None, kv_shift: int = 0, key_mask: Optional[torch.Tensor] = None,
              seq_index: Optional[torch.Tensor] = None):
    for n, t in (("q", q), ("k", k), ("v", v)):
        _rows2d(t, n)
    E = q.shape[1]
    if out is None:
        out = torch.empty(B * M, E, device=q.device, dtype=torch.float32)
    elif tuple(out.shape) != (B * M, E) or not out.is_contiguous() or out.dtype != torch.float32:
        raise ValueError("out must be a contiguous fp32 (B*M, E) tensor")
    if key_mask is not None:
        _chk(key_mask, torch.uint8, "key_mask")
        if tuple(key_mask.shape) != (B, N):
            raise ValueError(f"key_mask must be ({B}, {N}), got {tuple(key_mask.shape)}")
    if seq_index is not None:
        _chk(seq_index, torch.int32, "seq_index")
        if seq_index.numel() != B or key_mask is not None:
            raise ValueError("seq_index must hold B entries and excludes key_mask")
        _lib.check(_lib.load().dpm_attention_indexed(_ptr(q), q.stride(0), M * q.stride(0), _ptr(k), k.stride(0),
                                                     N * k.stride(0), _ptr(v), v.stride(0), N * v.stride(0), _ptr(out), E,
                                                     M * E, B, M, N, heads, E // heads, int(kv_shift), _ptr(seq_index),
                                                     _stream(q)), "dpm_attention_indexed")
        return out
    nsplit = attention_key_splits(B, M, N, heads, E // heads) if key_mask is None else 1
    if nsplit > 1:
        lib = _lib.load()
        ws = torch.empty(lib.dpm_attention_split_workspace_bytes(B, M, heads, E // heads, nsplit), device=q.device, dtype=torch.uint8)
        _lib.check(lib.dpm_attention_split(_ptr(q), q.stride(0), M * q.stride(0), _ptr(k), k.stride(0), N * k.stride(0),
                                           _ptr(v), v.stride(0), N * v.stride(0), _ptr(out), E, M * E, B, M, N, heads,
                                           E // heads, int(kv_shift), nsplit, _ptr(ws), _stream(q)), "dpm_attention_split")
        return out
    _lib.check(_lib.load().dpm_attention_masked(_ptr(q), q.stride(0), M * q.stride(0), _ptr(k), k.stride(0),
                                                N * k.stride(0), _ptr(v), v.stride(0), N * v.stride(0), _ptr(out), E,
                                                M * E, B, M, N, heads, E // heads, int(kv_shift), _ptr(key_mask), _stream(q)),
               "dpm_attention")
    return out


KV_PLANES_MIN_ROWS = 2048


def linear_kvplanes(x: torch.Tensor, W: torch.Tensor, bias: torch.Tensor, M: int, heads: int = 8):
    E = x.shape[-1]
    if (not knobs.KV_PLANES or not knobs.GEMM_BF16X3 or E != heads * 32 or M % 64 != 0 or tuple(W.shape) != (3 * E, E) or
            E > knobs.BF16X3_MAX_K or x.dim() != 2 or x.shape[0] % M != 0 or x.dtype != torch.float32 or not x.is_cuda or
            x.stride(1) != 1 or bias is None or bias.data_ptr() % 16 or x.shape[0] < KV_PLANES_MIN_ROWS):
        return None
    wp = _weight_planes(W)
    if wp is None:
        return None
    planes, off, n = wp
    U = x.shape[0] // M
    lib = _lib.load()
    q = torch.empty(U * M, E, device=x.device, dtype=torch.float32)
    kv = torch.empty(lib.dpm_attention_planes_bytes(U, M, heads), device=x.device, dtype=torch.uint8)
    st = lib.dpm_linear_bf16x3_kvplanes(_ptr(x), x.stride(0), planes.data_ptr() + 2 * off, E, n, _ptr(bias), _ptr(q), E, U * M, E, 3 * E, E,
                                        M, heads, _ptr(kv), _stream(x))
    if st == -2:
        return None
    _lib.check(st, "dpm_linear_bf16x3_kvplanes")
    return q, kv


def attention_planes(q: torch.Tensor, kv: torch.Tensor, B: int, M: int, heads: int = 8, kv_shift: int = 0,
                     seq_index: Optional[torch.Tensor] = None) -> torch.Tensor:
    E = q.shape[1]
    out = torch.empty(B * M, E, device=q.device, dtype=torch.float32)
    _lib.check(_lib.load().dpm_attention_planes(_ptr(q), E, M * E, _ptr(kv), _ptr(out), E, M * E, B, M, M, heads, int(kv_shift),
                                                _ptr(seq_index), _stream(q)), "dpm_attention_planes")
    return out


def qkv_attention(x: torch.Tensor, W: torch.Tensor, bias: torch.Tensor, B: int, M: int, heads: int = 8, kv_shift: int = 0,
                  seq_index: Optional[torch.Tensor] = None) -> Optional[torch.Tensor]:
    if x.dim() != 2 or M <= 0 or x.shape[0] % M != 0 or attention_key_splits(B, M, M, heads, 32) > 1:
        return None
    if seq_index is not None:
        _chk(seq_index, torch.int32, "seq_index")
        if seq_index.numel() != B:
            raise ValueError("seq_index must hold B entries")
    elif x.shape[0] // M != B:
        raise ValueError("x must hold B sequences when seq_index is not given")
    made = linear_kvplanes(x, W, bias, M, heads)
    if made is None:
        return None
    return attention_planes(made[0], made[1], B, M, heads, kv_shift, seq_index)


def l2_normalize(x: torch.Tensor) -> torch.Tensor:
    _chk(x, torch.float32, "x")
    out = torch.empty_like(x)
    _lib.check(_lib.load().dpm_l2_normalize(_ptr(x), x.numel() // x.shape[-1], x.shape[-1], _ptr(out), _stream(x)),
               "dpm_l2_normalize")
    return out


def dual_softmax_topk(S: torch.Tensor, tau: float, k: int):
    _chk(S, torch.float32, "S")
    single = S.dim() == 2
    B = 1 if single else S.shape[0]
    M, N = S.shape[-2], S.shape[-1]
    lib = _lib.load()
    val = torch.empty(B, k, device=S.device, dtype=torch.float32)
    idx = torch.empty(B, k, device=S.device, dtype=torch.int32)
    ws = torch.empty(lib.dpm_pairing_workspace_bytes(B, M, N), device=S.device, dtype=torch.uint8)
    _lib.check(lib.dpm_dual_softmax_topk(_ptr(S), B, M, N, float(tau), k, _ptr(val), _ptr(idx), _ptr(ws), _stream(S)),
               "dpm_dual_softmax_topk")
    return (val[0], idx[0]) if single else (val, idx)


# ... 1697 lines not shown
```

### include/dpm_hip.h

```cpp
#ifndef DPM_HIP_H
#define DPM_HIP_H

#include <stddef.h>
#include <stdint.h>

#ifdef __cplusplus
extern "C" {
#endif

typedef void *dpm_stream_t;

#define DPM_OK 0
#define DPM_EINVAL (-1)
#define DPM_EUNSUPPORTED (-2)

#define DPM_ACT_NONE 0
#define DPM_ACT_RELU 1
#define DPM_ACT_SIGMOID 2

#define DPM_VERSION_EXPERIMENT 0x40000000
int dpm_version(void);
const char *dpm_error_string(int status);

int dpm_prepare_points(const float *points_cf, const uint8_t *padding, int B, int C, int N,
                       float *xyz, int32_t *lengths, dpm_stream_t stream);

int dpm_to_channel_first(const float *x, int B, int R, int C, float *out, dpm_stream_t stream);
int dpm_to_channel_first_ld(const float *x, int B, int R, int C, float *out, int ldo, dpm_stream_t stream);

int dpm_emit_descriptors(const float *xyz, const float *fea, const int32_t *lengths, int B, int S, int C,
                         double coor_scale, float *coor, float *feat, uint8_t *padding, float *desc, dpm_stream_t stream);

int dpm_nested_levels(const float *xyz0, const int32_t *len0, int B, int K0, int n_levels, const int32_t *npoint,
                      float *xyz_out, int32_t *idx_out, int32_t *len_out, dpm_stream_t stream);

int dpm_gather_frames(const float *src, long long frame_stride, int rows, int ld, int cols, const int32_t *index, int n,
                      float *out, dpm_stream_t stream);

size_t dpm_fps_workspace_bytes(int B, int N, int K);
int dpm_fps(const float *xyz, const int32_t *lengths, int B, int N, int K, int32_t *idx,
            float *new_xyz, int32_t *new_lengths, void *workspace, dpm_stream_t stream);
int dpm_fps_ex(const float *xyz, const int32_t *lengths, int B, int N, int K, int32_t *idx,
               float *new_xyz, int32_t *new_lengths, void *workspace, int algo, dpm_stream_t stream);
int dpm_fps_start(const float *xyz, const int32_t *lengths, const int32_t *start, int B, int N, int K, int32_t *idx,
                  float *new_xyz, int32_t *new_lengths, void *workspace, dpm_stream_t stream);

size_t dpm_knn_workspace_bytes(int B, int N);
int dpm_knn_hybrid(const float *points, const int32_t *lengths, const float *centers, int B, int N,
                   int S, int K, double radius, int32_t *idx, void *workspace, dpm_stream_t stream);

int dpm_knn_hybrid_reuse(const float *points, const int32_t *lengths, const float *centers, int B, int N,
                         int S, int K, double radius, int32_t *idx, void *workspace, const int32_t *reuse_idx,
                         const int32_t *center_src, dpm_stream_t stream);

int dpm_knn_build_grid(const float *points, const int32_t *lengths, int B, int N, double radius, void *workspace,
                       dpm_stream_t stream);
int dpm_knn_hybrid_prebuilt(const float *points, const int32_t *lengths, const float *centers, int B, int N,
                            int S, int K, double radius, int32_t *idx, void *workspace, dpm_stream_t stream);

int dpm_ball_query(const float *points, const int32_t *lengths, const float *centers, int B, int N, int S,
                   int K, double radius, int32_t *idx, dpm_stream_t stream);

int dpm_voxel_sampler_bounds(const float *points, const uint8_t *padding, int B, int N, int D, double voxel_size,
                             double sample_range, float *hdr, dpm_stream_t stream);
size_t dpm_voxel_sampler_workspace_bytes(int B, int N, long long max_cells);
int dpm_voxel_sampler_select(const float *points, const uint8_t *padding, int B, int N, int D, double voxel_size,
                             double sample_range, float *hdr, long long max_cells, int K, int32_t *sel, int cap,
                             int32_t *n_unique, void *workspace, dpm_stream_t stream);


int dpm_posegraph_optimize(const double *poses, int n, const int32_t *src, const int32_t *dst, const double *X,
                           const double *info, int E, int reference_node, const double *criteria, double *out_poses,
                           double *stats);

int dpm_host_topk_replay(const float *values, int n, int k, int largest, int32_t *out_idx);
int dpm_host_sort_replay(const float *values, int n, int descending, int32_t *out_idx);

int dpm_group_mlp_max_generic(const float *xyz, const float *fea, const float *centers,
                              const int32_t *idx, const float *W, const float *bias, const float *gamma,
                              const float *beta, int B, int N, int S, int K, int Cin, int Cout, double radius,
                              float *out, dpm_stream_t stream);
int dpm_group_mlp_max(const float *xyz, const float *fea, const float *centers, const int32_t *idx,
                      const float *W, const float *bias, const float *gamma, const float *beta,
                      int B, int N, int S, int K, int Cin, int Cout, double radius, float *out,
                      dpm_stream_t stream);

int dpm_group_mlp_max_from_xyz(const float *xyz, const float *W0, const float *b0, const float *centers,
                               const int32_t *idx, const float *W, const float *bias, const float *gamma,
                               const float *beta, int B, int N, int S, int K, int Cin, int Cout,
                               double radius, float *out, dpm_stream_t stream);

int dpm_group_gather_ln_max(const float *P, const float *xyz, const float *centers, const int32_t *idx,
                            const float *W_rel, int ldw_rel, const float *gamma, const float *beta, int B, int N,
                            int S, int K, int Cout, double radius, float *out, dpm_stream_t stream);
int dpm_group_affine_ln_max(const float *A, const float *cvec, const float *xyz, const float *centers,
                            const int32_t *idx, const float *W_rel, int ldw_rel, const float *gamma,
                            const float *beta, int B, int N, int S, int K, int Cout, double radius, float *out,
                            dpm_stream_t stream);
int dpm_group_gather_ln_max_folded(const float *P, const float *centers, const int32_t *idx, const float *W_rel, int ldw_rel,
                                   const float *gamma, const float *beta, int B, int N, int S, int K, int Cout, double radius,
                                   float *out, dpm_stream_t stream);
int dpm_group_gather_ln_max_centred(const float *P, const float *centers, const int32_t *idx, const float *W_rel, int ldw_rel,
                                    const float *gamma, const float *beta, int B, int N, int S, int K, int Cout, double radius,
                                    float *out, dpm_stream_t stream);
int dpm_group_affine_ln_max_centred(const float *A, const float *cvec, const float *xyz, const float *centers,
                                    const int32_t *idx, const float *W_rel, int ldw_rel, const float *gamma,
                                    const float *beta, int B, int N, int S, int K, int Cout, double radius, float *out,
                                    dpm_stream_t stream);

int dpm_linear(const float *x, int ldx, const float *W, int ldw, const float *bias,
               const float *residual, int ldr, float *out, int ldo, int R, int Cin, int Cout, int act,
               dpm_stream_t stream);
int dpm_linear_batched(const float *x, int ldx, long long sx, const float *W, int ldw, long long sw,
                       const float *bias, const float *residual, int ldr, long long sr, float *out,
                       int ldo, long long so, int batch, int R, int Cin, int Cout, int act,
                       dpm_stream_t stream);

int dpm_layernorm(const float *x, int ldx, const float *pre, const float *gamma, const float *beta,
                  const float *post, float *out, int ldo, int R, int C, int act, dpm_stream_t stream);

int dpm_linear_layernorm(const float *x, int ldx, const float *W, int ldw, const float *bias, const float *pre,
                         const float *gamma, const float *beta, const float *post, float *out, int ldo, int R, int Cin,
                         int Cout, int act, dpm_stream_t stream);

int dpm_three_interp_cat(const float *xyz1, const float *xyz2, const int32_t *lengths2,
                         const float *fea1, const float *fea2, int B, int N, int S, int D1, int D2,
                         float *out, dpm_stream_t stream);


int dpm_posemb(const float *xyz, int ld, const float *dim_t, int F, int E, int R, float *out,
               dpm_stream_t stream);

int dpm_attention(const float *Q, int ldq, long long sq, const float *K, int ldk, long long sk,
                  const float *V, int ldv, long long sv, float *out, int ldo, long long so, int B, int M,
                  int N, int heads, int head_dim, dpm_stream_t stream);
int dpm_attention_shifted(const float *Q, int ldq, long long sq, const float *K, int ldk, long long sk,
                          const float *V, int ldv, long long sv, float *out, int ldo, long long so, int B, int M,
                          int N, int heads, int head_dim, int kv_shift, dpm_stream_t stream);

int dpm_attention_masked(const float *Q, int ldq, long long sq, const float *K, int ldk, long long sk,
                         const float *V, int ldv, long long sv, float *out, int ldo, long long so, int B, int M,
                         int N, int heads, int head_dim, int kv_shift, const uint8_t *key_mask, dpm_stream_t stream);

int dpm_attention_indexed(const float *Q, int ldq, long long sq, const float *K, int ldk, long long sk,
                          const float *V, int ldv, long long sv, float *out, int ldo, long long so, int B, int M,
                          int N, int heads, int head_dim, int kv_shift, const int32_t *seq_index, dpm_stream_t stream);

size_t dpm_attention_split_workspace_bytes(int B, int M, int heads, int head_dim, int nsplit);
int dpm_attention_split(const float *Q, int ldq, long long sq, const float *K, int ldk, long long sk, const float *V,
                        int ldv, long long sv, float *out, int ldo, long long so, int B, int M, int N, int heads,
                        int head_dim, int kv_shift, int nsplit, void *workspace, dpm_stream_t stream);

size_t dpm_attention_planes_bytes(int n_sequences, int N, int heads);
int dpm_linear_bf16x3_kvplanes(const float *x, int ldx, const void *w_planes, int ldw, long long plane_stride,
                               const float *bias, float *out, int ldo, int R, int Cin, int Cout, int kv_col0, int tokens,
                               int heads, void *kv_planes, dpm_stream_t stream);
int dpm_attention_planes(const float *Q, int ldq, long long sq, const void *kv_planes, float *out, int ldo, long long so,
                         int B, int M, int N, int heads, int kv_shift, const int32_t *seq_index, dpm_stream_t stream);

int dpm_split_bf16x3(const float *W, long long n, void *planes, dpm_stream_t stream);
int dpm_linear_bf16x3(const float *x, int ldx, const void *w_planes, int ldw, long long plane_stride, const float *bias,
                      const float *residual, int ldr, float *out, int ldo, int R, int Cin, int Cout, int act,
                      dpm_stream_t stream);
int dpm_linear_bf16x3_rank3(const float *x, int ldx, const void *w_planes, int ldw, long long plane_stride, const float *bias,
                            const float *residual, int ldr, float *out, int ldo, int R, int Cin, int Cout, int act,
                            const float *x3, const float *w3, int ldw3, double scale, dpm_stream_t stream);
int dpm_linear_layernorm_bf16x3(const float *x, int ldx, const void *w_planes, int ldw, long long plane_stride,
                                const float *bias, const float *pre, const float *gamma, const float *beta, const float *post,
                                float *out, int ldo, int R, int Cin, int Cout, int act, dpm_stream_t stream);

int dpm_decoder_tail_bf16x3(const float *a, const float *pre, const float *post, float *out, int R, int C, const void *wo_planes,
                            long long plane_stride_o, const float *bo, const float *gamma2, const float *beta2,
                            const void *w0_planes, long long plane_stride_0, const float *b0, const void *w2_planes,
                            long long plane_stride_2, const float *b2, const float *gamma3, const float *beta3,
                            dpm_stream_t stream);

int dpm_pwconv_pair_bf16x3(const float *x, int ldx, const void *w1_planes, long long plane_stride1, const float *b1,
                           const float *gamma1, const float *beta1, const void *w2_planes_kperm, long long plane_stride2,
                           const float *b2, const float *gamma2, const float *beta2, const float *post, float *out, int R,
                           int C, int H, dpm_stream_t stream);

int dpm_l2_normalize(const float *x, int R, int C, float *out, dpm_stream_t stream);

size_t dpm_match_workspace_bytes(int batch, int M, int N, int k);
int dpm_match_topk(const float *a, const float *b, int batch, int M, int N, int C, double tau, int k, float *out_val,
                   int32_t *out_idx, void *workspace, dpm_stream_t stream);

size_t dpm_pairing_workspace_bytes(int batch, int M, int N);
int dpm_dual_softmax_topk(float *S, int batch, int M, int N, double tau, int k, float *out_val,
                          int32_t *out_idx, void *workspace, dpm_stream_t stream);

int dpm_gather_pairs(const float *x, const float *y, const int32_t *flat_idx, int batch, int k, int M,
                     int N, int E, float *X, int32_t *src_idx, int32_t *dst_idx, dpm_stream_t stream);

int dpm_mean_rows(const float *x, int B, int R, int C, float *out, int ldo, dpm_stream_t stream);

size_t dpm_kabsch_workspace_bytes(int batch, int k);
int dpm_corr_kabsch(const float *offsets, const float *src_xyz, int ld_src, long long stride_src,
                    const float *dst_xyz, int ld_dst, long long stride_dst, const int32_t *src_idx,
                    const int32_t *dst_idx, const float *conf, int batch, int k, double eps_offset,
                    int num_iter, double std_ratio, void *workspace, float *result, float *header,
                    int header_stride, dpm_stream_t stream);


size_t dpm_preprocess_workspace_bytes(long long max_cells);
int dpm_preprocess_scan(const float *xyz, int N, int stride, double voxel_size, double min_dis, double max_dis,
                        double ratio, long long max_cells, float *out_xyz, int32_t *out_idx, int out_capacity,
                        int32_t *status, void *workspace, dpm_stream_t stream);

size_t dpm_knn_self_workspace_bytes(int N);
int dpm_knn_self(const float *xyz, int N, int K, double cell, int32_t *idx, float *dist2, float *mean_dist,
                 void *workspace, dpm_stream_t stream);
int dpm_point_normals(const float *xyz, int N, double radius, float *normals, void *workspace, dpm_stream_t stream);
int dpm_lowpass_similarity(const float *normals, const int32_t *idx, int N, int K, int flux, float *sim,
                           dpm_stream_t stream);
int dpm_stat_filter(const float *stat, int N, double k_std, int mode, double ratio, const float *xyz_in,
                    const int32_t *idx_in, float *xyz_out, int32_t *idx_out, int32_t *n_out, dpm_stream_t stream);

size_t dpm_filter_dc_workspace_bytes(int capacity, int K);
int dpm_outlier_filter_dc(const float *xyz, const int32_t *idx_in, const int32_t *count, int capacity, int nb_neighbors,
                          double std_ratio, double cell, double ratio, float *xyz_out, int32_t *idx_out,
                          int32_t *count_out, void *workspace, dpm_stream_t stream);
int dpm_lowpass_filter_dc(const float *xyz, const int32_t *idx_in, const int32_t *count, int capacity,
                          double normals_radius, int normals_num, double filter_std, int flux, double cell, double ratio,
                          float *xyz_out, int32_t *idx_out, int32_t *count_out, void *workspace, dpm_stream_t stream);


size_t dpm_augment_workspace_bytes(int capacity, long long cells);
int dpm_ground_filter(const float *xyz, const int32_t *idx_in, const int32_t *count, int capacity, int img_len,
                      int img_width, double grid_width, double ground_height, int preserve_sparse_ground, float *out_xyz,
                      int32_t *out_idx, int32_t *out_count, void *workspace, dpm_stream_t stream);
int dpm_voxel_select(const float *xyz, const int32_t *idx_in, const int32_t *count, int capacity, double voxel_size,
                     int retention, long long max_cells, float *out_xyz, int32_t *out_idx, int32_t *status,
                     void *workspace, dpm_stream_t stream);
int dpm_mask_select(const float *xyz, const int32_t *idx_in, const int32_t *count, int capacity, int use_distance,
                    double min_dis, double max_dis, const float *u, double drop_ratio, const float *wedges, int n_wedges,
                    float *out_xyz, int32_t *out_idx, int32_t *out_count, void *workspace, dpm_stream_t stream);
int dpm_points_affine(float *xyz, const int32_t *count, int capacity, int mode, const double *params,
                      const float *jitter, dpm_stream_t stream);
int dpm_gather_points(const float *xyz, const int32_t *idx_in, const int32_t *count, int capacity, const int32_t *sel,
                      int n_sel, int limit, float *out_xyz, int32_t *out_idx, int32_t *out_count, dpm_stream_t stream);
int dpm_points_deskew(float *xyz, const int32_t *idx, const int32_t *count, int capacity, int time_mode, const float *times,
                      int n_times, int azimuth_steps, const double *motion, double s_ref, dpm_stream_t stream);
int dpm_pack_frames(const float *const *xyz, const int32_t *const *counts, const int32_t *capacities, int S,
                    int padding_to, float *points, unsigned char *padding, int32_t *status, dpm_stream_t stream);


int dpm_ingest_frames(const void *staging_host, void *staging_dev, long long staging_bytes, int F, int capacity,
                      int chunk, float *xyz, int32_t *idx, int32_t *count, void *workspace, dpm_stream_t stream);


int dpm_map_tile(const float *key_points, const int32_t *select, const float *poses, const float *centering,
                 int C, int S, int K, float *out, dpm_stream_t stream);


size_t dpm_infomat_workspace_bytes(int n_pairs, int N1, int N2);
int dpm_information_matrix(const float *pcd1, int N1, const float *pcd2, int N2, const float *Rt,
                           double radius, float *out6x6, void *workspace, dpm_stream_t stream);
int dpm_information_matrix_batched(const float *pcd, int N, const int32_t *src_frame,
                                   const int32_t *dst_frame, int n_pairs, const float *Rt, int rt_stride,
                                   double radius, float *out, int out_stride, void *workspace,
                                   dpm_stream_t stream);
int dpm_infomat_build_grids(const float *pcd, int N, const int32_t *dst_frame, int n_pairs, double radius,
                            void *workspace, dpm_stream_t stream);
int dpm_infomat_search_grids(const float *pcd, int N, const int32_t *src_frame, const int32_t *dst_frame,
                             int n_pairs, const float *Rt, int rt_stride, double radius, float *out,
                             int out_stride, void *workspace, dpm_stream_t stream);


#define DPM_ICP_POINT 0
#define DPM_ICP_PLANE 1
#define DPM_ICP_CONVERGED 0
#define DPM_ICP_MAX_ITER 1
#define DPM_ICP_NO_MATCH 2
#define DPM_ICP_SINGULAR 3
size_t dpm_icp_workspace_bytes(int n_pairs, int N);
int dpm_icp_refine_batched(const float *pcd, int F, int N, const int32_t *lengths, const float *normals,
                           const int32_t *src_frame, const int32_t *dst_frame, int n_pairs, const double *init_pose,
                           int metric, const double *stage_max_dist, const int32_t *stage_max_iter, int n_stages,
                           double tol_rot, double tol_trans, double *pose, float *fitness, float *rmse,
                           int32_t *iterations, int32_t *status, int32_t *debug_match, double *debug_system,
                           void *workspace, dpm_stream_t stream);


size_t dpm_voxel_map_workspace_bytes(long long n_points);
int dpm_voxel_map_init(long long n_points, void *workspace, dpm_stream_t stream);
int dpm_voxel_map_bounds(const float *const *clouds, const long long *offsets, const float *poses, int n_scans,
                         long long n_batch, void *workspace, dpm_stream_t stream);
int dpm_voxel_map_insert(const float *const *clouds, const long long *offsets, const float *poses, int n_scans,
                         long long n_batch, long long base, long long n_points, double min_x, double min_y,
                         double min_z, double voxel_size, void *workspace, dpm_stream_t stream);
int dpm_voxel_map_finish(long long n_points, void *workspace, dpm_stream_t stream);
int dpm_voxel_map_emit(const void *workspace, long long n_points, double min_x, double min_y, double min_z,
                       double voxel_size, float *centroids, int32_t *counts, int M, dpm_stream_t stream);

int dpm_reg_loss_pairs(const float *xyz_a, const float *xyz_b, int B, int M, int N, double eps, int32_t *nn_a, int32_t *nn_b,
                       int32_t *neutral_a, int32_t *neutral_b, dpm_stream_t stream);
size_t dpm_reg_loss_workspace_bytes(int B, int M, int N, int C);
int dpm_reg_loss_forward(const float *fea_a, const float *fea_b, const float *xyz_a, const float *xyz_b, const uint8_t *pad_a,
                         const uint8_t *pad_b, const int32_t *nn_a, const int32_t *nn_b, int B, int M, int N, int C, double tau,
                         double eps, int neutral, int32_t *argmax_a, int32_t *argmax_b, float *loss, float *stats,
                         void *workspace, dpm_stream_t stream);
int dpm_reg_loss_backward(const float *xyz_a, const float *xyz_b, const int32_t *nn_a, const int32_t *nn_b, int B, int M, int N,
                          int C, double tau, double eps, int neutral, const float *grad_loss, const float *stats,
                          const void *workspace, float *grad_a, float *grad_b, dpm_stream_t stream);

size_t dpm_attention_train_workspace_bytes(int B, int M, int N, int heads);
int dpm_attention_train_forward(const float *Q, int ldq, long long sq, const float *K, int ldk, long long sk, const float *V,
                                int ldv, long long sv, float *out, int ldo, long long so, float *lse, int B, int M, int N,
                                int heads, int head_dim, const uint8_t *key_mask, dpm_stream_t stream);
int dpm_attention_train_backward(const float *Q, int ldq, long long sq, const float *K, int ldk, long long sk, const float *V,
                                 int ldv, long long sv, const float *out, int ldo, long long so, const float *lse,
                                 const float *dout, int ldd, long long sd, const uint8_t *key_mask, float *dQ, float *dK,
                                 float *dV, int B, int M, int N, int heads, int head_dim, void *workspace, dpm_stream_t stream);

int dpm_offset_pairs_count(const float *xyz_a, const float *xyz_b, const uint8_t *pad_a, const uint8_t *pad_b, int B, int M, int N,
                           double eps, int32_t *counts, int32_t *offsets, dpm_stream_t stream);
int dpm_offset_pairs_fill(const float *xyz_a, const float *xyz_b, const uint8_t *pad_a, const uint8_t *pad_b, int B, int M, int N,
                          double eps, const int32_t *offsets, int32_t *triples, dpm_stream_t stream);
int dpm_offset_pairs_gather(const float *x, int ldx, const int32_t *triples, int side, int rows, long long K, int E, float *out,
                            dpm_stream_t stream);
int dpm_offset_pairs_segment_sum(const float *g, int ldg, const int32_t *offsets, const int32_t *perm, long long R, int E,
                                 float *out, dpm_stream_t stream);

int dpm_group_train_forward(const float *P, const float *xyz, const float *centers, const int32_t *idx, const float *W_rel,
                            int ldw_rel, const float *gamma, const float *beta, int B, int N, int S, int K, int Cout,
                            double radius, float *out, uint8_t *slots, dpm_stream_t stream);
size_t dpm_group_train_workspace_bytes(int B, int N, int S, int K, int Cout);
// ... 166 lines not shown
```

Before: 16450 frames/s.

## Fuse similarity head and offset head MLP chains into single bf16x3 kernels

Adds two fused kernels for the registration heads. One runs the similarity head (two 256x256 linears with ReLU, then L2 normalize) in a single launch. The other gathers matched pairs and runs the offset-head MLP chain plus the downsample residual in one launch, leaving only the final head linear separate. Shared bf16x3 chain helpers move into a common header. The aim is to cut kernel launches and the global-memory round trips of intermediate activations, at the cost of more specialised code paths that only apply when E=256.

After: 16570 frames/s, median of 6. About the same (+0.7%).

```diff
diff --git a/deeppointmap_amd/_lib.py b/deeppointmap_amd/_lib.py
--- a/deeppointmap_amd/_lib.py
+++ b/deeppointmap_amd/_lib.py
@@ -53,6 +53,8 @@
     "dpm_linear_layernorm_bf16x3": (I, [P, I, P, I, LL, P, P, P, P, P, P, I, I, I, I, I, P]),
     "dpm_pwconv_pair_bf16x3": (I, [P, I, P, LL, P, P, P, P, LL, P, P, P, P, P, I, I, I, P]),
     "dpm_decoder_tail_bf16x3": (I, [P, P, P, P, I, I, P, LL, P, P, P, P, LL, P, P, LL, P, P, P, P]),
+    "dpm_similarity_head_bf16x3": (I, [P, P, I, I, P, LL, P, P, LL, P, P]),
+    "dpm_offset_head_bf16x3": (I, [P, P, P, I, I, I, I, I, P, LL, P, P, LL, P, P, LL, P, P, LL, P, P, P, P, P]),
     "dpm_layernorm": (I, [P, I, P, P, P, P, P, I, I, I, I, P]),
     "dpm_linear_layernorm": (I, [P, I, P, I, P, P, P, P, P, P, I, I, I, I, I, P]),
     "dpm_three_interp_cat": (I, [P, P, P, P, P, I, I, I, I, I, P, P]),
diff --git a/deeppointmap_amd/csrc/b3_chain.h b/deeppointmap_amd/csrc/b3_chain.h
--- /dev/null
+++ b/deeppointmap_amd/csrc/b3_chain.h
@@ -0,0 +1,172 @@
+#pragma once
+#include "dpm_common.h"
+#include <type_traits>
+
+namespace {
+
+using bf16x8 = __attribute__((ext_vector_type(8))) __bf16;
+using f32x4 = __attribute__((ext_vector_type(4))) float;
+using u32x4 = __attribute__((ext_vector_type(4))) unsigned;
+using u32x2 = __attribute__((ext_vector_type(2))) unsigned;
+
+constexpr int B3_KT = 32, B3_LD = B3_KT;
+
+constexpr int DT_BM = 64, DT_C = 256, DT_T = 512, DT_NK = DT_C / B3_KT, DT_LDC = DT_C + 4;
+#ifndef DPM_TAIL_STASH
+#define DPM_TAIL_STASH 2
+#endif
+constexpr int DT_NS = DPM_TAIL_STASH, DT_OPER = 3 * (DT_BM + DT_C) * B3_LD;
+__device__ __forceinline__ f32x4 *dt_stash(uint16_t *smem, int kt) {
+    return reinterpret_cast<f32x4 *>(smem + DT_OPER) + (kt - (DT_NK - DT_NS)) * DT_T + threadIdx.x;
+}
+__device__ __forceinline__ void dt_stash_put(uint16_t *smem, const f32x4 (&v)[DT_NK]) {
+#pragma unroll
+    for (int kt = DT_NK - DT_NS; kt < DT_NK; ++kt) *dt_stash(smem, kt) = v[kt];
+}
+
+template <typename V, typename P>
+__device__ __forceinline__ V *dt_at(P *uniform, unsigned bytes) {
+    using B = std::conditional_t<std::is_const<P>::value, const char, char>;
+    return reinterpret_cast<V *>(reinterpret_cast<B *>(uniform) + bytes);
+}
+__device__ __forceinline__ long long dt_uniform(long long o) {
+    const unsigned lo = __builtin_amdgcn_readfirstlane((unsigned)o), hi = __builtin_amdgcn_readfirstlane((unsigned)((unsigned long long)o >> 32));
+    return (long long)(((unsigned long long)hi << 32) | lo);
+}
+template <int CTRL>
+__device__ __forceinline__ float dt_dpp(float v) {
+    return __int_as_float(__builtin_amdgcn_update_dpp(__float_as_int(v), __float_as_int(v), CTRL, 0xF, 0xF, false));
+}
+__device__ __forceinline__ float dt_row_sum(float (&s)[DT_NK]) {
+#pragma unroll
+    for (int kt = 0; kt < DT_NK; ++kt) {
+        s[kt] += dt_dpp<0xB1>(s[kt]);
+        s[kt] += dt_dpp<0x4E>(s[kt]);
+        s[kt] += dt_dpp<0x141>(s[kt]);
+    }
+    return ((s[0] + s[1]) + (s[2] + s[3])) + ((s[4] + s[5]) + (s[6] + s[7]));
+}
+__device__ __forceinline__ void dt_layernorm(f32x4 (&v)[DT_NK], const float *__restrict__ gamma, const float *__restrict__ beta, int sk) {
+    float s[DT_NK];
+#pragma unroll
+    for (int kt = 0; kt < DT_NK; ++kt) s[kt] = (v[kt][0] + v[kt][1]) + (v[kt][2] + v[kt][3]);
+    const float mu = dt_row_sum(s) / (float)DT_C;
+#pragma unroll
+    for (int kt = 0; kt < DT_NK; ++kt) {
+        v[kt][0] -= mu, v[kt][1] -= mu, v[kt][2] -= mu, v[kt][3] -= mu;
+        s[kt] = fmaf(v[kt][0], v[kt][0], fmaf(v[kt][1], v[kt][1], fmaf(v[kt][2], v[kt][2], v[kt][3] * v[kt][3])));
+    }
+    const float rs = rsqrtf(dt_row_sum(s) / (float)DT_C + 1e-5f);
+#pragma unroll
+    for (int kt = 0; kt < DT_NK; ++kt) {
+        const f32x4 g4 = *reinterpret_cast<const f32x4 *>(gamma + kt * B3_KT + sk), b4 = *reinterpret_cast<const f32x4 *>(beta + kt * B3_KT + sk);
+#pragma unroll
+        for (int q = 0; q < 4; ++q) v[kt][q] = fmaf(v[kt][q] * rs, g4[q], b4[q]);
+    }
+}
+
+__device__ __forceinline__ const u32x4 *dt_wsrc(const uint16_t *__restrict__ Wp, long long plane, int p, int pl, int k0, unsigned wo) {
+    return dt_at<const u32x4>(Wp + dt_uniform(pl * plane + p * (DT_T / 4) * DT_C) + k0, wo);
+}
+__device__ __forceinline__ unsigned dt_woff() { return (unsigned)((threadIdx.x >> 2) * DT_C + (threadIdx.x & 3) * 8) * 2u; }
+__device__ __forceinline__ void dt_wtile0(const uint16_t *__restrict__ Wp, long long plane, u32x4 (&wv)[2][3]) {
+    const unsigned wo = dt_woff();
+#pragma unroll
+    for (int p = 0; p < 2; ++p)
+#pragma unroll
+        for (int pl = 0; pl < 3; ++pl) wv[p][pl] = *dt_wsrc(Wp, plane, p, pl, 0, wo);
+}
+
+template <bool XREG, typename Mid>
+__device__ __forceinline__ void dt_product(uint16_t *smem, const float *xg, unsigned xo, const f32x4 (&xr)[DT_NK], const uint16_t *__restrict__ Wp,
+                                           long long plane, u32x4 (&wv)[2][3], f32x4 (&acc)[2][4], Mid mid) {
+    constexpr int WM = 32, WN = 64, MB = 2, NB = 4, PW = 2;
+    uint16_t (*Xs)[DT_BM][B3_LD] = reinterpret_cast<uint16_t (*)[DT_BM][B3_LD]>(smem);
+    uint16_t (*Ws)[DT_C][B3_LD] = reinterpret_cast<uint16_t (*)[DT_C][B3_LD]>(smem + 3 * DT_BM * B3_LD);
+    const int t = threadIdx.x, lane = t & 63, w = t >> 6, wm = w >> 2, wn = w & 3;
+    const int sr = t >> 3, sk = (t & 7) * 4, wk = (t & 3) * 8, fr = lane & 15, fk = (lane >> 4) * 8;
+    const int wrow = t >> 2;
+    const unsigned wo = dt_woff();
+    f32x4 xv = f32x4{0.f, 0.f, 0.f, 0.f};
+    if (!XREG) xv = *dt_at<const f32x4>(xg, xo);
+#pragma unroll
+    for (int i = 0; i < MB; ++i)
+#pragma unroll
+        for (int j = 0; j < NB; ++j) acc[i][j] = f32x4{0.f, 0.f, 0.f, 0.f};
+#pragma unroll
+    for (int kt = 0; kt < DT_NK; ++kt) {
+        {
+            const f32x4 x = !XREG ? xv : kt >= DT_NK - DT_NS ? *dt_stash(smem, kt) : xr[kt];
+            unsigned h0, m0, l0, h1, m1, l1, h2, m2, l2, h3, m3, l3;
+            split3(x[0], h0, m0, l0), split3(x[1], h1, m1, l1), split3(x[2], h2, m2, l2), split3(x[3], h3, m3, l3);
+            *reinterpret_cast<u32x2 *>(&Xs[0][sr][b3_col(sr, sk)]) = u32x2{pack2(h0, h1), pack2(h2, h3)};
+            *reinterpret_cast<u32x2 *>(&Xs[1][sr][b3_col(sr, sk)]) = u32x2{pack2(m0, m1), pack2(m2, m3)};
+            *reinterpret_cast<u32x2 *>(&Xs[2][sr][b3_col(sr, sk)]) = u32x2{pack2(l0, l1), pack2(l2, l3)};
+        }
+#pragma unroll
+        for (int p = 0; p < PW; ++p)
+#pragma unroll
+            for (int pl = 0; pl < 3; ++pl) *reinterpret_cast<u32x4 *>(&Ws[pl][p * (DT_T / 4) + wrow][b3_col(wrow, wk)]) = wv[p][pl];
+        __syncthreads();
+        if (kt + 1 < DT_NK) {
+            const int kn = (kt + 1) * B3_KT;
+            unsigned wok = wo;
+            asm volatile("" : "+v"(wok));
+            if (!XREG) xv = *dt_at<const f32x4>(xg + kn, xo);
+#pragma unroll
+            for (int p = 0; p < PW; ++p)
+#pragma unroll
+                for (int pl = 0; pl < 3; ++pl) wv[p][pl] = *dt_wsrc(Wp, plane, p, pl, kn, wok);
+        }
+        mid(kt);
+        bf16x8 b[3][MB];
+#pragma unroll
+        for (int pl = 0; pl < 3; ++pl)
+#pragma unroll
+            for (int i = 0; i < MB; ++i) b[pl][i] = *reinterpret_cast<const bf16x8 *>(&Xs[pl][wm * WM + i * 16 + fr][b3_col(fr, fk)]);
+#pragma unroll
+        for (int j = 0; j < NB; ++j) {
+            bf16x8 a[3];
+#pragma unroll
+            for (int pl = 0; pl < 3; ++pl) a[pl] = *reinterpret_cast<const bf16x8 *>(&Ws[pl][wn * WN + j * 16 + fr][b3_col(fr, fk)]);
+#define DPM_B3(PWQ, PXQ) \
+    _Pragma("unroll") for (int i = 0; i < MB; ++i) acc[i][j] = __builtin_amdgcn_mfma_f32_16x16x32_bf16(a[PWQ], b[PXQ][i], acc[i][j], 0, 0, 0)
+            DPM_B3(1, 1);
+            DPM_B3(2, 0);
+            DPM_B3(0, 2);
+            DPM_B3(1, 0);
+            DPM_B3(0, 1);
+            DPM_B3(0, 0);
+#undef DPM_B3
+        }
+        __syncthreads();
+    }
+}
+
+template <typename Mid>
+__device__ __forceinline__ void dt_restage(uint16_t *smem, const f32x4 (&acc)[2][4], f32x4 (&v)[DT_NK], Mid mid) {
+    float *ct = reinterpret_cast<float *>(smem);
+    int t = threadIdx.x;
+    asm volatile("" : "+v"(t));
+    const int lane = t & 63, w = t >> 6, wm = w >> 2, wn = w & 3, sr = t >> 3, sk = (t & 7) * 4;
+#pragma unroll
+    for (int i = 0; i < 2; ++i)
+#pragma unroll
+        for (int j = 0; j < 4; ++j)
+            *reinterpret_cast<f32x4 *>(&ct[(wm * 32 + i * 16 + (lane & 15)) * DT_LDC + wn * 64 + j * 16 + (lane >> 4) * 4]) = acc[i][j];
+    mid();
+    __syncthreads();
+#pragma unroll
+    for (int kt = 0; kt < DT_NK; ++kt) v[kt] = *reinterpret_cast<const f32x4 *>(&ct[sr * DT_LDC + kt * B3_KT + sk]);
+    __syncthreads();
+}
+
+__device__ __forceinline__ void dt_add_bias(f32x4 (&v)[DT_NK], const float *__restrict__ bias, int sk) {
+#pragma unroll
+    for (int kt = 0; kt < DT_NK; ++kt) {
+        const f32x4 bv = bias ? *reinterpret_cast<const f32x4 *>(bias + kt * B3_KT + sk) : f32x4{0.f, 0.f, 0.f, 0.f};
+        v[kt] += bv;
+    }
+}
+
+}
diff --git a/deeppointmap_amd/csrc/build.py b/deeppointmap_amd/csrc/build.py
--- a/deeppointmap_amd/csrc/build.py
+++ b/deeppointmap_amd/csrc/build.py
@@ -16,6 +16,7 @@
     "encoder_ops.hip": [],
     "gemm.hip": [],
     "gemm_b3.hip": [],
+    "reg_heads.hip": [],
     "group_mlp.hip": [],
     "decoder_ops.hip": [],
     "match.hip": [],
diff --git a/deeppointmap_amd/csrc/gemm_b3.hip b/deeppointmap_amd/csrc/gemm_b3.hip
--- a/deeppointmap_amd/csrc/gemm_b3.hip
+++ b/deeppointmap_amd/csrc/gemm_b3.hip
@@ -1,12 +1,6 @@
-#include "dpm_common.h"
-#include <type_traits>
+#include "b3_chain.h"
 
 namespace {
-
-using bf16x8 = __attribute__((ext_vector_type(8))) __bf16;
-using f32x4 = __attribute__((ext_vector_type(4))) float;
-using u32x4 = __attribute__((ext_vector_type(4))) unsigned;
-using u32x2 = __attribute__((ext_vector_type(2))) unsigned;
 
 __device__ __forceinline__ float b3_act(float v, int act) {
     if (act == DPM_ACT_RELU) return fmaxf(v, 0.f);
@@ -28,7 +22,6 @@
 #ifndef DPM_B3_DEEP
 #define DPM_B3_DEEP 256
 #endif
-constexpr int B3_KT = 32, B3_LD = B3_KT;
 
 struct KvPlanes {
     uint16_t *p;
@@ -385,163 +378,6 @@
     const float *g2, *be2, *g3, *be3;
     int R;
 };
-constexpr int DT_BM = 64, DT_C = 256, DT_T = 512, DT_NK = DT_C / B3_KT, DT_LDC = DT_C + 4;
-#ifndef DPM_TAIL_STASH
-#define DPM_TAIL_STASH 2
-#endif
-constexpr int DT_NS = DPM_TAIL_STASH, DT_OPER = 3 * (DT_BM + DT_C) * B3_LD;
-__device__ __forceinline__ f32x4 *dt_stash(uint16_t *smem, int kt) {
-    return reinterpret_cast<f32x4 *>(smem + DT_OPER) + (kt - (DT_NK - DT_NS)) * DT_T + threadIdx.x;
-}
-__device__ __forceinline__ void dt_stash_put(uint16_t *smem, const f32x4 (&v)[DT_NK]) {
-#pragma unroll
-    for (int kt = DT_NK - DT_NS; kt < DT_NK; ++kt) *dt_stash(smem, kt) = v[kt];
-}
-
-template <typename V, typename P>
-__device__ __forceinline__ V *dt_at(P *uniform, unsigned bytes) {
-    using B = std::conditional_t<std::is_const<P>::value, const char, char>;
-    return reinterpret_cast<V *>(reinterpret_cast<B *>(uniform) + bytes);
-}
-__device__ __forceinline__ long long dt_uniform(long long o) {
-    const unsigned lo = __builtin_amdgcn_readfirstlane((unsigned)o), hi = __builtin_amdgcn_readfirstlane((unsigned)((unsigned long long)o >> 32));
-    return (long long)(((unsigned long long)hi << 32) | lo);
-}
-template <int CTRL>
-__device__ __forceinline__ float dt_dpp(float v) {
-    return __int_as_float(__builtin_amdgcn_update_dpp(__float_as_int(v), __float_as_int(v), CTRL, 0xF, 0xF, false));
-}
-__device__ __forceinline__ float dt_row_sum(float (&s)[DT_NK]) {
-#pragma unroll
-    for (int kt = 0; kt < DT_NK; ++kt) {
-        s[kt] += dt_dpp<0xB1>(s[kt]);
-        s[kt] += dt_dpp<0x4E>(s[kt]);
-        s[kt] += dt_dpp<0x141>(s[kt]);
-    }
-    return ((s[0] + s[1]) + (s[2] + s[3])) + ((s[4] + s[5]) + (s[6] + s[7]));
-}
-__device__ __forceinline__ void dt_layernorm(f32x4 (&v)[DT_NK], const float *__restrict__ gamma, const float *__restrict__ beta, int sk) {
-    float s[DT_NK];
-#pragma unroll
-    for (int kt = 0; kt < DT_NK; ++kt) s[kt] = (v[kt][0] + v[kt][1]) + (v[kt][2] + v[kt][3]);
-    const float mu = dt_row_sum(s) / (float)DT_C;
-#pragma unroll
-    for (int kt = 0; kt < DT_NK; ++kt) {
-        v[kt][0] -= mu, v[kt][1] -= mu, v[kt][2] -= mu, v[kt][3] -= mu;
-        s[kt] = fmaf(v[kt][0], v[kt][0], fmaf(v[kt][1], v[kt][1], fmaf(v[kt][2], v[kt][2], v[kt][3] * v[kt][3])));
-    }
-    const float rs = rsqrtf(dt_row_sum(s) / (float)DT_C + 1e-5f);
-#pragma unroll
-    for (int kt = 0; kt < DT_NK; ++kt) {
-        const f32x4 g4 = *reinterpret_cast<const f32x4 *>(gamma + kt * B3_KT + sk), b4 = *reinterpret_cast<const f32x4 *>(beta + kt * B3_KT + sk);
-#pragma unroll
-        for (int q = 0; q < 4; ++q) v[kt][q] = fmaf(v[kt][q] * rs, g4[q], b4[q]);
-    }
-}
-
-__device__ __forceinline__ const u32x4 *dt_wsrc(const uint16_t *__restrict__ Wp, long long plane, int p, int pl, int k0, unsigned wo) {
-    return dt_at<const u32x4>(Wp + dt_uniform(pl * plane + p * (DT_T / 4) * DT_C) + k0, wo);
-}
-__device__ __forceinline__ unsigned dt_woff() { return (unsigned)((threadIdx.x >> 2) * DT_C + (threadIdx.x & 3) * 8) * 2u; }
-__device__ __forceinline__ void dt_wtile0(const uint16_t *__restrict__ Wp, long long plane, u32x4 (&wv)[2][3]) {
-    const unsigned wo = dt_woff();
-#pragma unroll
-    for (int p = 0; p < 2; ++p)
-#pragma unroll
-        for (int pl = 0; pl < 3; ++pl) wv[p][pl] = *dt_wsrc(Wp, plane, p, pl, 0, wo);
-}
-
-template <bool XREG, typename Mid>
-__device__ __forceinline__ void dt_product(uint16_t *smem, const float *xg, unsigned xo, const f32x4 (&xr)[DT_NK], const uint16_t *__restrict__ Wp,
-                                           long long plane, u32x4 (&wv)[2][3], f32x4 (&acc)[2][4], Mid mid) {
-    constexpr int WM = 32, WN = 64, MB = 2, NB = 4, PW = 2;
-    uint16_t (*Xs)[DT_BM][B3_LD] = reinterpret_cast<uint16_t (*)[DT_BM][B3_LD]>(smem);
-    uint16_t (*Ws)[DT_C][B3_LD] = reinterpret_cast<uint16_t (*)[DT_C][B3_LD]>(smem + 3 * DT_BM * B3_LD);
-    const int t = threadIdx.x, lane = t & 63, w = t >> 6, wm = w >> 2, wn = w & 3;
-    const int sr = t >> 3, sk = (t & 7) * 4, wk = (t & 3) * 8, fr = lane & 15, fk = (lane >> 4) * 8;
-    const int wrow = t >> 2;
-    const unsigned wo = dt_woff();
-    f32x4 xv = f32x4{0.f, 0.f, 0.f, 0.f};
-    if (!XREG) xv = *dt_at<const f32x4>(xg, xo);
-#pragma unroll
-    for (int i = 0; i < MB; ++i)
-#pragma unroll
-        for (int j = 0; j < NB; ++j) acc[i][j] = f32x4{0.f, 0.f, 0.f, 0.f};
-#pragma unroll
-    for (int kt = 0; kt < DT_NK; ++kt) {
-        {
-            const f32x4 x = !XREG ? xv : kt >= DT_NK - DT_NS ? *dt_stash(smem, kt) : xr[kt];
-            unsigned h0, m0, l0, h1, m1, l1, h2, m2, l2, h3, m3, l3;
-            split3(x[0], h0, m0, l0), split3(x[1], h1, m1, l1), split3(x[2], h2, m2, l2), split3(x[3], h3, m3, l3);
-            *reinterpret_cast<u32x2 *>(&Xs[0][sr][b3_col(sr, sk)]) = u32x2{pack2(h0, h1), pack2(h2, h3)};
-            *reinterpret_cast<u32x2 *>(&Xs[1][sr][b3_col(sr, sk)]) = u32x2{pack2(m0, m1), pack2(m2, m3)};
-            *reinterpret_cast<u32x2 *>(&Xs[2][sr][b3_col(sr, sk)]) = u32x2{pack2(l0, l1), pack2(l2, l3)};
-        }
-#pragma unroll
-        for (int p = 0; p < PW; ++p)
-#pragma unroll
-            for (int pl = 0; pl < 3; ++pl) *reinterpret_cast<u32x4 *>(&Ws[pl][p * (DT_T / 4) + wrow][b3_col(wrow, wk)]) = wv[p][pl];
-        __syncthreads();
-        if (kt + 1 < DT_NK) {
-            const int kn = (kt + 1) * B3_KT;
-            unsigned wok = wo;
-            asm volatile("" : "+v"(wok));
-            if (!XREG) xv = *dt_at<const f32x4>(xg + kn, xo);
-#pragma unroll
-            for (int p = 0; p < PW; ++p)
-#pragma unroll
-                for (int pl = 0; pl < 3; ++pl) wv[p][pl] = *dt_wsrc(Wp, plane, p, pl, kn, wok);
-        }
-        mid(kt);
-        bf16x8 b[3][MB];
-#pragma unroll
-        for (int pl = 0; pl < 3; ++pl)
-#pragma unroll
-            for (int i = 0; i < MB; ++i) b[pl][i] = *reinterpret_cast<const bf16x8 *>(&Xs[pl][wm * WM + i * 16 + fr][b3_col(fr, fk)]);
-#pragma unroll
-        for (int j = 0; j < NB; ++j) {
-            bf16x8 a[3];
-#pragma unroll
-            for (int pl = 0; pl < 3; ++pl) a[pl] = *reinterpret_cast<const bf16x8 *>(&Ws[pl][wn * WN + j * 16 + fr][b3_col(fr, fk)]);
-#define DPM_B3(PWQ, PXQ) \
-    _Pragma("unroll") for (int i = 0; i < MB; ++i) acc[i][j] = __builtin_amdgcn_mfma_f32_16x16x32_bf16(a[PWQ], b[PXQ][i], acc[i][j], 0, 0, 0)
-            DPM_B3(1, 1);
-            DPM_B3(2, 0);
-            DPM_B3(0, 2);
-            DPM_B3(1, 0);
-            DPM_B3(0, 1);
-            DPM_B3(0, 0);
-#undef DPM_B3
-        }
-        __syncthreads();
-    }
-}
-
-template <typename Mid>
-__device__ __forceinline__ void dt_restage(uint16_t *smem, const f32x4 (&acc)[2][4], f32x4 (&v)[DT_NK], Mid mid) {
-    float *ct = reinterpret_cast<float *>(smem);
-    int t = threadIdx.x;
-    asm volatile("" : "+v"(t));
-    const int lane = t & 63, w = t >> 6, wm = w >> 2, wn = w & 3, sr = t >> 3, sk = (t & 7) * 4;
-#pragma unroll
-    for (int i = 0; i < 2; ++i)
-#pragma unroll
-        for (int j = 0; j < 4; ++j)
-            *reinterpret_cast<f32x4 *>(&ct[(wm * 32 + i * 16 + (lane & 15)) * DT_LDC + wn * 64 + j * 16 + (lane >> 4) * 4]) = acc[i][j];
-    mid();
-    __syncthreads();
-#pragma unroll
-    for (int kt = 0; kt < DT_NK; ++kt) v[kt] = *reinterpret_cast<const f32x4 *>(&ct[sr * DT_LDC + kt * B3_KT + sk]);
-    __syncthreads();
-}
-
-__device__ __forceinline__ void dt_add_bias(f32x4 (&v)[DT_NK], const float *__restrict__ bias, int sk) {
-#pragma unroll
-    for (int kt = 0; kt < DT_NK; ++kt) {
-        const f32x4 bv = bias ? *reinterpret_cast<const f32x4 *>(bias + kt * B3_KT + sk) : f32x4{0.f, 0.f, 0.f, 0.f};
-        v[kt] += bv;
-    }
-}
 
 template <bool ZREG>
 __global__ __launch_bounds__(DT_T) __attribute__((amdgpu_waves_per_eu(4, 4))) void decoder_tail_b3_kernel(TailArgs A) {
diff --git a/deeppointmap_amd/csrc/reg_heads.hip b/deeppointmap_amd/csrc/reg_heads.hip
--- /dev/null
+++ b/deeppointmap_amd/csrc/reg_heads.hip
@@ -0,0 +1,274 @@
+#include "b3_chain.h"
+
+namespace {
+
+struct SimArgs {
+    const float *x;
+    float *out;
+    const uint16_t *w[2];
+    long long plane[2];
+    const float *bias[2];
+    int R;
+};
+__global__ __launch_bounds__(DT_T) __attribute__((amdgpu_waves_per_eu(4, 4))) void sim_head_b3_kernel(SimArgs A) {
+    constexpr int SM0 = DT_OPER + DT_NS * DT_T * 8, SM1 = 2 * DT_BM * DT_LDC, SM = SM0 > SM1 ? SM0 : SM1;
+    __shared__ __attribute__((aligned(16))) uint16_t smem[SM];
+    const int t = threadIdx.x, sr = t >> 3, sk = (t & 7) * 4;
+    const int row0 = blockIdx.x * DT_BM;
+    const long long base = dt_uniform((long long)row0 * DT_C);
+    const unsigned ro = (unsigned)(min(sr, A.R - 1 - row0) * DT_C + sk) * 4u;
+    f32x4 acc[2][4], v[DT_NK];
+    u32x4 wv[2][3];
+    dt_wtile0(A.w[0], A.plane[0], wv);
+    dt_product<false>(smem, A.x + base, ro, v, A.w[0], A.plane[0], wv, acc, [](int) {});
+    dt_restage(smem, acc, v, [&] { dt_wtile0(A.w[1], A.plane[1], wv); });
+    dt_add_bias(v, A.bias[0], sk);
+#pragma unroll
+    for (int kt = 0; kt < DT_NK; ++kt)
+#pragma unroll
+        for (int q = 0; q < 4; ++q) v[kt][q] = fmaxf(v[kt][q], 0.f);
+    dt_stash_put(smem, v);
+    dt_product<true>(smem, nullptr, 0u, v, A.w[1], A.plane[1], wv, acc, [](int) {});
+    float *ct = reinterpret_cast<float *>(smem);
+    {
+        const int lane = t & 63, w = t >> 6, wm = w >> 2, wn = w & 3;
+#pragma unroll
+        for (int i = 0; i < 2; ++i)
+#pragma unroll
+            for (int j = 0; j < 4; ++j)
+                *reinterpret_cast<f32x4 *>(&ct[(wm * 32 + i * 16 + (lane & 15)) * DT_LDC + wn * 64 + j * 16 + (lane >> 4) * 4]) = acc[i][j];
+    }
+    __syncthreads();
+    const int lane = t & 63, w = t >> 6;
+    float bl[4];
+#pragma unroll
+    for (int q = 0; q < 4; ++q) bl[q] = A.bias[1] ? A.bias[1][lane + 64 * q] : 0.f;
+    const f32x4 b4 = A.bias[1] ? *reinterpret_cast<const f32x4 *>(A.bias[1] + lane * 4) : f32x4{0.f, 0.f, 0.f, 0.f};
+    float *gout = A.out + base;
+#pragma unroll 2
+    for (int i = 0; i < DT_BM / 8; ++i) {
+        const int rr = w * (DT_BM / 8) + i;
+        if (row0 + rr >= A.R) break;
+        const float *c = ct + rr * DT_LDC;
+        float s = 0.f;
+#pragma unroll
+        for (int q = 0; q < 4; ++q) {
+            const float e = c[lane + 64 * q] + bl[q];
+            s = fmaf(e, e, s);
+        }
+        const float nrm = fmaxf(sqrtf(wave_sum(s)), 1e-12f);
+        f32x4 o = *reinterpret_cast<const f32x4 *>(c + lane * 4) + b4;
+        o[0] /= nrm, o[1] /= nrm, o[2] /= nrm, o[3] /= nrm;
+        *reinterpret_cast<f32x4 *>(gout + rr * DT_C + lane * 4) = o;
+    }
+}
+
+struct OffsetArgs {
+    const float *x, *y;
+    const int32_t *flat;
+    const uint16_t *w[4];
+    long long plane[4];
+    const float *bias[4];
+    float *out;
+    int32_t *si, *di;
+    int B, k, M, N;
+};
+constexpr int OH_T = 512, OH_BM = 64, OH_E = 256;
+
+template <int NK, int WROWS, int NB, bool UNROLL, typename XAt, typename WAt, typename Col>
+__device__ __forceinline__ void oh_product(uint16_t *smem, XAt xat, WAt wat, Col col, f32x4 (&acc)[2][NB]) {
+    constexpr int PW = (WROWS * 4 + OH_T - 1) / OH_T;
+    uint16_t (*Xs)[OH_BM][B3_LD] = reinterpret_cast<uint16_t (*)[OH_BM][B3_LD]>(smem);
+    uint16_t (*Ws)[WROWS][B3_LD] = reinterpret_cast<uint16_t (*)[WROWS][B3_LD]>(smem + 3 * OH_BM * B3_LD);
+    const int t = threadIdx.x, lane = t & 63, wm = t >> 8;
+    const int sr = t >> 3, sk = (t & 7) * 4, wrow = t >> 2, wk = (t & 3) * 8, fr = lane & 15, fk = (lane >> 4) * 8;
+    f32x4 xv = xat(0);
+    u32x4 wv[PW][3];
+#pragma unroll
+    for (int p = 0; p < PW; ++p)
+#pragma unroll
+        for (int pl = 0; pl < 3; ++pl) wv[p][pl] = *wat(p, pl, 0);
+#pragma unroll
+    for (int i = 0; i < 2; ++i)
+#pragma unroll
+        for (int j = 0; j < NB; ++j) acc[i][j] = f32x4{0.f, 0.f, 0.f, 0.f};
+    auto step = [&](int kt) {
+        {
+            unsigned h0, m0, l0, h1, m1, l1, h2, m2, l2, h3, m3, l3;
+            split3(xv[0], h0, m0, l0), split3(xv[1], h1, m1, l1), split3(xv[2], h2, m2, l2), split3(xv[3], h3, m3, l3);
+            *reinterpret_cast<u32x2 *>(&Xs[0][sr][b3_col(sr, sk)]) = u32x2{pack2(h0, h1), pack2(h2, h3)};
+            *reinterpret_cast<u32x2 *>(&Xs[1][sr][b3_col(sr, sk)]) = u32x2{pack2(m0, m1), pack2(m2, m3)};
+            *reinterpret_cast<u32x2 *>(&Xs[2][sr][b3_col(sr, sk)]) = u32x2{pack2(l0, l1), pack2(l2, l3)};
+        }
+#pragma unroll
+        for (int p = 0; p < PW; ++p) {
+            if ((p + 1) * (OH_T / 4) <= WROWS || p * (OH_T / 4) + wrow < WROWS) {
+#pragma unroll
+                for (int pl = 0; pl < 3; ++pl) *reinterpret_cast<u32x4 *>(&Ws[pl][p * (OH_T / 4) + wrow][b3_col(wrow, wk)]) = wv[p][pl];
+            }
+        }
+        __syncthreads();
+        {
+            const int kn = min(kt + 1, NK - 1);
+            xv = xat(kn);
+#pragma unroll
+            for (int p = 0; p < PW; ++p)
+#pragma unroll
+                for (int pl = 0; pl < 3; ++pl) wv[p][pl] = *wat(p, pl, kn);
+        }
+        bf16x8 b[3][2];
+#pragma unroll
+        for (int pl = 0; pl < 3; ++pl)
+#pragma unroll
+            for (int i = 0; i < 2; ++i) b[pl][i] = *reinterpret_cast<const bf16x8 *>(&Xs[pl][wm * 32 + i * 16 + fr][b3_col(fr, fk)]);
+#pragma unroll
+        for (int j = 0; j < NB; ++j) {
+            bf16x8 a[3];
+#pragma unroll
+            for (int pl = 0; pl < 3; ++pl) a[pl] = *reinterpret_cast<const bf16x8 *>(&Ws[pl][col(j) + fr][b3_col(fr, fk)]);
+#define DPM_B3(PWQ, PXQ) \
+    _Pragma("unroll") for (int i = 0; i < 2; ++i) acc[i][j] = __builtin_amdgcn_mfma_f32_16x16x32_bf16(a[PWQ], b[PXQ][i], acc[i][j], 0, 0, 0)
+            DPM_B3(1, 1);
+            DPM_B3(2, 0);
+            DPM_B3(0, 2);
+            DPM_B3(1, 0);
+            DPM_B3(0, 1);
+            DPM_B3(0, 0);
+#undef DPM_B3
+        }
+        __syncthreads();
+    };
+    if constexpr (UNROLL) {
+#pragma unroll
+        for (int kt = 0; kt < NK; ++kt) step(kt);
+    } else {
+#pragma unroll 1
+        for (int kt = 0; kt < NK; ++kt) step(kt);
+    }
+}
+
+template <int NB, int NK, typename Col>
+__device__ __forceinline__ void oh_restage(uint16_t *smem, const f32x4 (&acc)[2][NB], Col col, f32x4 (&v)[NK]) {
+    constexpr int LDC = NK * B3_KT + 4;
+    float *ct = reinterpret_cast<float *>(smem);
+    const int t = threadIdx.x, lane = t & 63, wm = t >> 8, sr = t >> 3, sk = (t & 7) * 4;
+#pragma unroll
+    for (int i = 0; i < 2; ++i)
+#pragma unroll
+        for (int j = 0; j < NB; ++j) *reinterpret_cast<f32x4 *>(&ct[(wm * 32 + i * 16 + (lane & 15)) * LDC + col(j) + (lane >> 4) * 4]) = acc[i][j];
+    __syncthreads();
+#pragma unroll
+    for (int kt = 0; kt < NK; ++kt) v[kt] = *reinterpret_cast<const f32x4 *>(&ct[sr * LDC + kt * B3_KT + sk]);
+    __syncthreads();
+}
+
+template <int NK>
+__device__ __forceinline__ void oh_bias_relu(f32x4 (&v)[NK], const float *__restrict__ bias, int sk) {
+#pragma unroll
+    for (int kt = 0; kt < NK; ++kt) {
+        const f32x4 bv = bias ? *reinterpret_cast<const f32x4 *>(bias + kt * B3_KT + sk) : f32x4{0.f, 0.f, 0.f, 0.f};
+        v[kt] += bv;
+#pragma unroll
+        for (int q = 0; q < 4; ++q) v[kt][q] = fmaxf(v[kt][q], 0.f);
+    }
+}
+
+__global__ __launch_bounds__(OH_T) __attribute__((amdgpu_waves_per_eu(4, 4))) void offset_head_b3_kernel(OffsetArgs A) {
+    constexpr int C0 = OH_E, C2 = OH_E / 2, C4 = OH_E / 4, K0 = 2 * OH_E;
+    constexpr int SM0 = 3 * (OH_BM + C0 + C4) * B3_LD, SM1 = 2 * OH_BM * (C0 + 4), SM = SM0 > SM1 ? SM0 : SM1;
+    __shared__ __attribute__((aligned(16))) uint16_t smem[SM];
+    const int t = threadIdx.x, lane = t & 63, w = t >> 6, wm = w >> 2, wn = w & 3, sr = t >> 3, sk = (t & 7) * 4;
+    const int row0 = blockIdx.x * OH_BM, rows = A.B * 2 * A.k;
+    const float *xa, *xb;
+    {
+        const int g = min(row0 + sr, rows - 1), b = g / (2 * A.k), q = g - b * 2 * A.k, p = q < A.k ? q : q - A.k;
+        const int f = A.flat[(size_t)b * A.k + p];
+        const int si = f / A.N, di = f - si * A.N;
+        const float *xs = A.x + ((size_t)b * A.M + si) * OH_E + sk, *yd = A.y + ((size_t)b * A.N + di) * OH_E + sk;
+        xa = q < A.k ? xs : yd, xb = q < A.k ? yd : xs;
+        if ((t & 7) == 0 && q < A.k && row0 + sr < rows) A.si[(size_t)b * A.k + p] = si, A.di[(size_t)b * A.k + p] = di;
+    }
+    const int wr = t >> 2, wk = (t & 3) * 8;
+    f32x4 acc1[2][5];
+    const unsigned w0o = (unsigned)(wr * K0 + wk) * 2u, wdo = (unsigned)((wr & (C4 - 1)) * K0 + wk) * 2u;
+    oh_product<K0 / B3_KT, C0 + C4, 5, false>(
+        smem, [&](int kt) { return *reinterpret_cast<const f32x4 *>(kt < OH_E / B3_KT ? xa + kt * B3_KT : xb + (kt * B3_KT - OH_E)); },
+        [&](int p, int pl, int kt) {
+            return p < 2 ? dt_at<const u32x4>(A.w[0] + dt_uniform(pl * A.plane[0] + (long long)p * (OH_T / 4) * K0 + kt * B3_KT), w0o)
+                         : dt_at<const u32x4>(A.w[3] + dt_uniform(pl * A.plane[3] + kt * B3_KT), wdo);
+        },
+        [&](int j) { return j < 4 ? wn * 64 + j * 16 : C0 + wn * 16; }, acc1);
+    f32x4 d[2] = {acc1[0][4], acc1[1][4]};
+    f32x4 v1[C0 / B3_KT];
+    {
+        f32x4 a4[2][4];
+#pragma unroll
+        for (int i = 0; i < 2; ++i)
+#pragma unroll
+            for (int j = 0; j < 4; ++j) a4[i][j] = acc1[i][j];
+        oh_restage<4, C0 / B3_KT>(smem, a4, [&](int j) { return wn * 64 + j * 16; }, v1);
+    }
+    oh_bias_relu(v1, A.bias[0], sk);
+    f32x4 acc2[2][2];
+    const unsigned w2o = (unsigned)(wr * C0 + wk) * 2u;
+    oh_product<C0 / B3_KT, C2, 2, true>(
+        smem, [&](int kt) { return v1[kt]; },
+        [&](int, int pl, int kt) { return dt_at<const u32x4>(A.w[1] + dt_uniform(pl * A.plane[1] + kt * B3_KT), w2o); },
+        [&](int j) { return wn * 32 + j * 16; }, acc2);
+    f32x4 v2[C2 / B3_KT];
+    oh_restage<2, C2 / B3_KT>(smem, acc2, [&](int j) { return wn * 32 + j * 16; }, v2);
+    oh_bias_relu(v2, A.bias[1], sk);
+    f32x4 acc3[2][1];
+    const unsigned w4o = (unsigned)((wr & (C4 - 1)) * C2 + wk) * 2u;
+    oh_product<C2 / B3_KT, C4, 1, true>(
+        smem, [&](int kt) { return v2[kt]; },
+        [&](int, int pl, int kt) { return dt_at<const u32x4>(A.w[2] + dt_uniform(pl * A.plane[2] + kt * B3_KT), w4o); },
+        [&](int) { return wn * 16; }, acc3);
+    const int c = wn * 16 + (lane >> 4) * 4;
+    const f32x4 b4 = A.bias[2] ? *reinterpret_cast<const f32x4 *>(A.bias[2] + c) : f32x4{0.f, 0.f, 0.f, 0.f};
+    const f32x4 bd = A.bias[3] ? *reinterpret_cast<const f32x4 *>(A.bias[3] + c) : f32x4{0.f, 0.f, 0.f, 0.f};
+#pragma unroll
+    for (int i = 0; i < 2; ++i) {
+        const int r = row0 + wm * 32 + i * 16 + (lane & 15);
+        f32x4 o = (acc3[i][0] + b4) + (d[i] + bd);
+#pragma unroll
+        for (int q = 0; q < 4; ++q) o[q] = fmaxf(o[q], 0.f);
+        if (r < rows) *reinterpret_cast<f32x4 *>(A.out + (size_t)r * C4 + c) = o;
+    }
+}
+
+}
+
+extern "C" int dpm_similarity_head_bf16x3(const float *x, float *out, int R, int C, const void *w0_planes, long long plane_0,
+                                          const float *b0, const void *w2_planes, long long plane_2, const float *b2,
+                                          dpm_stream_t stream) {
+    DPM_CHECK_ARG(x && out && w0_planes && w2_planes && R >= 1 && C >= 1 && x != out);
+    const long long cc = (long long)C * C;
+    DPM_CHECK_ARG(plane_0 >= cc && plane_2 >= cc);
+    auto al = [](const void *p) { return ((uintptr_t)p & 15) == 0; };
+    if (C != DT_C || plane_0 % 8 != 0 || plane_2 % 8 != 0 || !al(x) || !al(out) || !al(w0_planes) || !al(w2_planes) || !al(b0) || !al(b2))
+        return DPM_EUNSUPPORTED;
+    const SimArgs A{x, out, {(const uint16_t *)w0_planes, (const uint16_t *)w2_planes}, {plane_0, plane_2}, {b0, b2}, R};
+    hipLaunchKernelGGL(sim_head_b3_kernel, dim3(dpm_cdiv(R, DT_BM)), dim3(DT_T), 0, (hipStream_t)stream, A);
+    return dpm_launch_status();
+}
+
+extern "C" int dpm_offset_head_bf16x3(const float *x, const float *y, const int32_t *flat_idx, int batch, int k, int M, int N, int E,
+                                      const void *w0_planes, long long plane_0, const float *b0, const void *w2_planes,
+                                      long long plane_2, const float *b2, const void *w4_planes, long long plane_4, const float *b4,
+                                      const void *wd_planes, long long plane_d, const float *bd, float *h_out, int32_t *src_idx,
+                                      int32_t *dst_idx, dpm_stream_t stream) {
+    DPM_CHECK_ARG(x && y && flat_idx && h_out && src_idx && dst_idx && w0_planes && w2_planes && w4_planes && wd_planes);
+    DPM_CHECK_ARG(batch >= 1 && k >= 1 && M >= 1 && N >= 1 && E >= 1 && (long long)batch * 2 * k <= 0x7fffffffLL);
+    const long long e = E;
+    DPM_CHECK_ARG(plane_0 >= 2 * e * e && plane_2 >= e * e / 2 && plane_4 >= e * e / 8 && plane_d >= e * e / 2);
+    auto al = [](const void *p) { return ((uintptr_t)p & 15) == 0; };
+    if (E != OH_E || plane_0 % 8 != 0 || plane_2 % 8 != 0 || plane_4 % 8 != 0 || plane_d % 8 != 0 || !al(x) || !al(y) || !al(h_out) ||
+        !al(w0_planes) || !al(w2_planes) || !al(w4_planes) || !al(wd_planes) || !al(b0) || !al(b2) || !al(b4) || !al(bd))
+        return DPM_EUNSUPPORTED;
+    const OffsetArgs A{x, y, flat_idx,
+                       {(const uint16_t *)w0_planes, (const uint16_t *)w2_planes, (const uint16_t *)w4_planes, (const uint16_t *)wd_planes},
+                       {plane_0, plane_2, plane_4, plane_d}, {b0, b2, b4, bd}, h_out, src_idx, dst_idx, batch, k, M, N};
+    hipLaunchKernelGGL(offset_head_b3_kernel, dim3(dpm_cdiv((long long)batch * 2 * k, OH_BM)), dim3(OH_T), 0, (hipStream_t)stream, A);
+    return dpm_launch_status();
+}
diff --git a/deeppointmap_amd/decoder.py b/deeppointmap_amd/decoder.py
--- a/deeppointmap_amd/decoder.py
+++ b/deeppointmap_amd/decoder.py
@@ -80,6 +80,13 @@
             return out
         z2 = self._lin_ln(ca, n2, a, z1)
         return self._lin_ln(m2, n3, self._lin(m0, z2, ops.ACT_RELU), z2, post)
+
+    def _similarity_head(self, z):
+        out = ops.similarity_head(z, self.p("similarity_head.0.weight"), self.p("similarity_head.0.bias"),
+                                  self.p("similarity_head.2.weight"), self.p("similarity_head.2.bias"))
+        if out is not None:
+            return out
+        return ops.l2_normalize(self._lin("similarity_head.2", self._lin("similarity_head.0", z, ops.ACT_RELU)))
 
     def _stage(self, desc: torch.Tensor, dev) -> Tuple[torch.Tensor, torch.Tensor, int, int]:
         d = desc.to(device=dev, dtype=torch.float32).contiguous()
@@ -350,21 +357,26 @@
                 x.untyped_storage().data_ptr() == y.untyped_storage().data_ptr() and
                 y.storage_offset() == x.storage_offset() + x.numel()):
             z = x.as_strided((2 * B * M, E), (E, 1), x.storage_offset())
-            ab = ops.l2_normalize(self._lin("similarity_head.2", self._lin("similarity_head.0", z, ops.ACT_RELU)))
+            ab = self._similarity_head(z)
             a, b = ab[:B * M], ab[B * M:]
         else:
-            a = ops.l2_normalize(self._lin("similarity_head.2", self._lin("similarity_head.0", x, ops.ACT_RELU)))
-            b = ops.l2_normalize(self._lin("similarity_head.2", self._lin("similarity_head.0", y, ops.ACT_RELU)))
+            a, b = self._similarity_head(x), self._similarity_head(y)
         if self.fused_match and ops.match_supported(M, N, E, k):
             conf, flat = ops.match_topk(a.view(B, M, E), b.view(B, N, E), self.tau, k)
         else:
             S = ops.similarity_batched(a.view(B, M, E), b.view(B, N, E))
             conf, flat = ops.dual_softmax_topk(S, self.tau, k)
-        X, si, di = ops.gather_pairs(x.view(B, M, E), y.view(B, N, E), flat)
-        X = X.view(B * 2 * k, 2 * E)
-        h = self._lin("offset_head.mlp.2", self._lin("offset_head.mlp.0", X, ops.ACT_RELU), ops.ACT_RELU)
-        h = self._lin("offset_head.mlp.4", h, ops.ACT_RELU, residual=self._lin("offset_head.downsample", X))
-        off = self._lin("offset_head.head", h)
+        oh = "offset_head."
+        fused = ops.offset_head(x.view(B, M, E), y.view(B, N, E), flat,
+                                *(self.p(oh + l + s) for l in ("mlp.0", "mlp.2", "mlp.4", "downsample", "head") for s in (".weight", ".bias")))
+        if fused is not None:
+            off, si, di = fused
+        else:
+            X, si, di = ops.gather_pairs(x.view(B, M, E), y.view(B, N, E), flat)
+            X = X.view(B * 2 * k, 2 * E)
+            h = self._lin("offset_head.mlp.2", self._lin("offset_head.mlp.0", X, ops.ACT_RELU), ops.ACT_RELU)
+            h = self._lin("offset_head.mlp.4", h, ops.ACT_RELU, residual=self._lin("offset_head.downsample", X))
+            off = self._lin("offset_head.head", h)
         res = ops.corr_kabsch(off, xyz_s, xyz_d, si, di, conf, self.args.loss.eps_offset, header_out=header_out, batch=B)
         if trace is not None:
             trace.update(x=x, y=y, conf=conf, flat=flat, src_index=si, dst_index=di, offsets=off)
diff --git a/deeppointmap_amd/knobs.py b/deeppointmap_amd/knobs.py
--- a/deeppointmap_amd/knobs.py
+++ b/deeppointmap_amd/knobs.py
@@ -16,10 +16,13 @@
 FUSED_MATCH = True
 KV_PLANES = True
 DECODER_TAIL_FUSED = True
+SIM_HEAD_FUSED = True
+OFFSET_HEAD_FUSED = True
 DEDUP_FRAMES = True
 
 _ENV = {"DPM_FOLD_MIN_RADIUS": ("FOLD_MIN_RADIUS", float), "DPM_KV_PLANES": ("KV_PLANES", lambda v: v != "0"), "DPM_CENTRED_GATHER": ("CENTRED_GATHER", lambda v: v != "0"), "DPM_FPS_ALGO": ("FPS_ALGO", int), "DPM_NO_FUSED_LN": ("FUSED_LN", lambda v: v != "1"),
-        "DPM_DEDUP_FRAMES": ("DEDUP_FRAMES", lambda v: v != "0"), "DPM_DECODER_TAIL": ("DECODER_TAIL_FUSED", lambda v: v != "0"), "DPM_GEMM_BF16X3": ("GEMM_BF16X3", lambda v: v == "1"), "DPM_BF16X3_MAX_K": ("BF16X3_MAX_K", int), "DPM_BF16X3_LN_MIN_K": ("BF16X3_LN_MIN_K", int), "DPM_FUSED_LN_SMALL_ROWS": ("FUSED_LN_SMALL_ROWS", int), "DPM_GEMM_LN_BF16X3": ("GEMM_LN_BF16X3", lambda v: v == "1"),
+        "DPM_DEDUP_FRAMES": ("DEDUP_FRAMES", lambda v: v != "0"), "DPM_DECODER_TAIL": ("DECODER_TAIL_FUSED", lambda v: v != "0"), "DPM_SIM_HEAD": ("SIM_HEAD_FUSED", lambda v: v != "0"), "DPM_OFFSET_HEAD": ("OFFSET_HEAD_FUSED", lambda v: v != "0"),
+        "DPM_GEMM_BF16X3": ("GEMM_BF16X3", lambda v: v == "1"), "DPM_BF16X3_MAX_K": ("BF16X3_MAX_K", int), "DPM_BF16X3_LN_MIN_K": ("BF16X3_LN_MIN_K", int), "DPM_FUSED_LN_SMALL_ROWS": ("FUSED_LN_SMALL_ROWS", int), "DPM_GEMM_LN_BF16X3": ("GEMM_LN_BF16X3", lambda v: v == "1"),
         "DPM_FUSED_MATCH": ("FUSED_MATCH", lambda v: v != "0"), "DPM_FUSED_PWCONV": ("FUSED_PWCONV", lambda v: v != "0"), "DPM_FOLD_GATHER": ("FOLD_GATHER", lambda v: v != "0")}
 
 
diff --git a/deeppointmap_amd/ops.py b/deeppointmap_amd/ops.py
--- a/deeppointmap_amd/ops.py
+++ b/deeppointmap_amd/ops.py
@@ -608,6 +608,60 @@
     return out
 
 
+def similarity_head(z: torch.Tensor, W0, b0, W2, b2) -> Optional[torch.Tensor]:
+    C = z.shape[-1]
+    if not (knobs.SIM_HEAD_FUSED and knobs.GEMM_BF16X3 and C == 256 and C <= knobs.BF16X3_MAX_K and z.is_cuda
+            and z.dtype == torch.float32 and z.dim() == 2 and z.is_contiguous() and z.shape[0] >= 1):
+        return None
+    planes = []
+    for W, b in ((W0, b0), (W2, b2)):
+        if tuple(W.shape[:2]) != (C, C) or W.numel() != C * C or (b is not None and b.data_ptr() % 16):
+            return None
+        wp = _weight_planes(W)
+        if wp is None:
+            return None
+        planes.append(wp)
+    R = z.shape[0]
+    out = torch.empty(R, C, device=z.device, dtype=torch.float32)
+    (p0, o0, n0), (p2, o2, n2) = planes
+    st = _lib.load().dpm_similarity_head_bf16x3(_ptr(z), _ptr(out), R, C, p0.data_ptr() + 2 * o0, n0, _ptr(b0),
+                                                p2.data_ptr() + 2 * o2, n2, _ptr(b2), _stream(z))
+    if st == -2:
+        return None
+    _lib.check(st, "dpm_similarity_head_bf16x3")
+    return out
+
+
+def offset_head(x: torch.Tensor, y: torch.Tensor, flat: torch.Tensor, W0, b0, W2, b2, W4, b4, Wd, bd, Wh, bh):
+    if not (knobs.OFFSET_HEAD_FUSED and knobs.GEMM_BF16X3 and x.dim() == 3 and y.dim() == 3 and flat.dim() == 2):
+        return None
+    B, M, E = x.shape
+    N, k = y.shape[1], flat.shape[1]
+    if not (E == 256 and 2 * E <= knobs.BF16X3_MAX_K and B >= 1 and k >= 1 and y.shape[0] == B and y.shape[2] == E and flat.shape[0] == B
+            and all(t_.is_cuda and t_.is_contiguous() for t_ in (x, y, flat)) and x.dtype == torch.float32 and y.dtype == torch.float32
+            and flat.dtype == torch.int32):
+        return None
+    planes = []
+    for W, b, shape in ((W0, b0, (E, 2 * E)), (W2, b2, (E // 2, E)), (W4, b4, (E // 4, E // 2)), (Wd, bd, (E // 4, 2 * E))):
+        if tuple(W.shape[:2]) != shape or W.numel() != shape[0] * shape[1] or (b is not None and b.data_ptr() % 16):
+            return None
+        wp = _weight_planes(W)
+        if wp is None:
+            return None
+        planes.append(wp)
+    h = torch.empty(B * 2 * k, E // 4, device=x.device, dtype=torch.float32)
+    si = torch.empty(B, k, device=x.device, dtype=torch.int32)
+    di = torch.empty(B, k, device=x.device, dtype=torch.int32)
+    (p0, o0, n0), (p2, o2, n2), (p4, o4, n4), (pd, od, nd) = planes
+    st = _lib.load().dpm_offset_head_bf16x3(_ptr(x), _ptr(y), _ptr(flat), B, k, M, N, E, p0.data_ptr() + 2 * o0, n0, _ptr(b0),
+                                            p2.data_ptr() + 2 * o2, n2, _ptr(b2), p4.data_ptr() + 2 * o4, n4, _ptr(b4),
+                                            pd.data_ptr() + 2 * od, nd, _ptr(bd), _ptr(h), _ptr(si), _ptr(di), _stream(x))
+    if st == -2:
+        return None
+    _lib.check(st, "dpm_offset_head_bf16x3")
+    return linear(h, Wh, bh), si, di
+
+
 def three_interp_cat(xyz1, xyz2, lengths2, fea1, fea2) -> torch.Tensor:
     for n, t in (("xyz1", xyz1), ("xyz2", xyz2), ("fea1", fea1), ("fea2", fea2)):
         _chk(t, torch.float32, n)
diff --git a/include/dpm_hip.h b/include/dpm_hip.h
--- a/include/dpm_hip.h
+++ b/include/dpm_hip.h
@@ -174,6 +174,16 @@
                             const void *w0_planes, long long plane_stride_0, const float *b0, const void *w2_planes,
                             long long plane_stride_2, const float *b2, const float *gamma3, const float *beta3,
                             dpm_stream_t stream);
+
+int dpm_similarity_head_bf16x3(const float *x, float *out, int R, int C, const void *w0_planes, long long plane_stride_0,
+                               const float *b0, const void *w2_planes, long long plane_stride_2, const float *b2,
+                               dpm_stream_t stream);
+
+int dpm_offset_head_bf16x3(const float *x, const float *y, const int32_t *flat_idx, int batch, int k, int M, int N, int E,
+                           const void *w0_planes, long long plane_stride_0, const float *b0, const void *w2_planes,
+                           long long plane_stride_2, const float *b2, const void *w4_planes, long long plane_stride_4,
+                           const float *b4, const void *wd_planes, long long plane_stride_d, const float *bd, float *h_out,
+                           int32_t *src_idx, int32_t *dst_idx, dpm_stream_t stream);
 
 int dpm_pwconv_pair_bf16x3(const float *x, int ldx, const void *w1_planes, long long plane_stride1, const float *b1,
                            const float *gamma1, const float *beta1, const void *w2_planes_kperm, long long plane_stride2,
```
